# marbl/MHAP

Measured on AMD Instinct MI355X. Metric: overlaps/sec, higher is better.
Workload: dtype int64

## Files before the change

mhap_amd/csrc/kernels.hpp:

```cpp
#pragma once
#include "device_common.hpp"

namespace mhap {

constexpr int HASH_TILE = 1024;
constexpr int WEIGHT_THREADS = 1024;
constexpr int WEIGHT_MAXIT = 24;
constexpr int MH_U = 4;
constexpr int ORD_THREADS = 256;
constexpr int ORD_BINS = 2048;
constexpr int CAND_TQ = 128;
constexpr int CAND_TM = 128;
constexpr int CAND_KS = 32;
constexpr int OVL_THREADS = 128;
#ifndef MH_INV_CT
#define MH_INV_CT 2048
#endif
constexpr int INV_CT = MH_INV_CT;

constexpr int BS_WCLASSES = 6;
constexpr int BS_WMAX = 32;
struct StrandInfo { int32_t valid; int32_t mode; int32_t cnt[BS_WCLASSES + 1]; int32_t pad; };

struct FilterTable {
  const int64_t* keys;
  const double* vals;
  uint32_t mask;
  uint32_t size;
  int32_t enabled;
  int32_t no_tf;
  double range;
  const unsigned long long* bloom; uint64_t bloom_bits; int32_t bloom_k; int32_t bloom_mode;
};

constexpr int META_W = 4;

struct Candidate { int32_t q; int32_t m; };

struct DevRecord { int32_t q, m; double score; int32_t raw, a1, a2, b1, b2, pad; };

struct SearchParams {
  int32_t H, S, k2;
  int32_t num_min_matches, min_store_length;
  int32_t to_self;
  int32_t own_queries;
  double max_shift, threshold;
};

void launch_hash_kmers(hipStream_t st, const ReadDesc* descs, int64_t nstrands, int max_len, const uint8_t* store, int64_t* keys,
                       int32_t* h32, int k, int k2, const uint64_t* luts, int only_mat);
void build_kmer_hash_luts(uint64_t* out);
int weight_grid(int num_cus, int64_t nstrands, int max_len, int k);
bool strand_hashes_from_codes(int length, int k, int k2);
void launch_kmer_weights(hipStream_t st, int num_cus, const ReadDesc* descs, int64_t nstrands, int max_len, const int64_t* keys,
                         uint32_t* wts, uint32_t* perm, uint32_t* slabs, int64_t slab_entries, unsigned long long* counter, int k,
                         const FilterTable& ft, double repeat_weight, StrandInfo* info, bool fused, const uint8_t* store,
                         const uint64_t* luts, const int32_t* order, int32_t* slist);
bool launch_minhash(hipStream_t st, hipStream_t st_weighted, int nblocks, int64_t n_unweighted, int64_t n_weighted, const ReadDesc* descs, int64_t nstrands, const int64_t* keys, const uint32_t* wts,
                    const uint32_t* perm, const StrandInfo* info, const uint8_t* store, const uint64_t* luts, int k, int k2, int H,
                    unsigned long long* counter, int32_t* out_rows, int64_t out_stride, int32_t* out_status, int64_t status_stride,
                    const uint64_t* jump, int jump_na, const int32_t* slist, uint32_t* qbuf, const uint64_t* unjump, const uint64_t* jump_w1, unsigned long long* merge,
                    int max_nk);
size_t minhash_merge_bytes(int nblocks, int H);
void build_xorshift_unjump_tables(int na, int nq, uint64_t* out);
int minhash_wgs_per_cu(int H);
size_t minhash_queue_bytes(int nblocks_total, int H);
int minhash_queue_words(int H);
constexpr int XS_JUMP_LOG2 = 2;
constexpr int XS_JUMP_NQ = BS_WMAX;
#ifndef MH_W1_JUMP_NA
#define MH_W1_JUMP_NA 16
#endif
constexpr int W1_JUMP_NA = MH_W1_JUMP_NA;
inline int w1_jump_tables(int H) { return W1_JUMP_NA + ((H + 1) >> XS_JUMP_LOG2) / W1_JUMP_NA + 1; }
void build_xorshift_jump_tables(int na, int nq, uint64_t* out);
void launch_fix_status(hipStream_t st, int32_t* meta, int64_t nreads);
size_t ordered_lds_bytes(int cap, int code_words, int stage_wide);
void launch_ordered(hipStream_t st, const ReadDesc* descs, int64_t nstrands, int max_len_codes, int max_len, const int32_t* h32,
                    const uint8_t* store, const uint64_t* luts, int k2, int S, int cap, int32_t* out_rows, int64_t out_stride,
                    int32_t* out_meta, int64_t meta_stride, int64_t first = 0, int64_t count = -1);

void launch_candidates(hipStream_t st, const int32_t* minhash, int64_t row_stride, const int32_t* qminhash, int64_t qrow_stride,
                       const int32_t* qlist, int nq, int ne, const int64_t* ids, const int64_t* qids, const int32_t* meta,
                       const int32_t* qmeta, const SearchParams& sp, const long long* rowstart, long long nblocks_tri, Candidate* cand,
                       unsigned long long* cand_count, unsigned long long cand_cap);
constexpr int MHAP_MAX_NUM_HASHES = 8192;
int minhash_waves_per_workgroup(int H);
struct InvIndex {
  uint32_t* ends;
  uint2* items;
  uint32_t nb, shift;
  uint64_t slot_stride;
  uint32_t ne;
  uint32_t grouped;
  uint32_t group_t, class_log;
  uint32_t* lines;
  uint32_t nl_log, line_lb, line_ebits;
  uint32_t tile_entries, tiles;
  uint2* staged;
  uint32_t* tile_counts;
  uint32_t* bin_start;
  uint32_t* bin_long;
};
void launch_query_iota(hipStream_t st, int32_t* qlist, int first, int n);
int index_tile_entries(int ne);
void index_group_params(int64_t entries, InvIndex& ix);
int index_coarse_bins();
bool index_line_params(int64_t entries, uint32_t nb, uint32_t& nl_log, uint32_t& lb, uint32_t& ebits);
size_t index_line_bytes(int H, uint32_t nl_log);
int index_max_buckets_log();
void launch_index_verify(hipStream_t st, const int32_t* minhash, int64_t row_stride, const int32_t* meta, int ne, int H, const InvIndex& ix,
                         unsigned long long* missing);
bool launch_index_build(hipStream_t st, const int32_t* minhash, int64_t row_stride, const int32_t* meta, int ne, int H, const InvIndex& ix);
void launch_index_query(hipStream_t st, const InvIndex& ix, const int32_t* qminhash, int64_t qrow_stride,
                        const int32_t* qlist, int nq, const int64_t* ids, const int64_t* qids, const int32_t* meta, const int32_t* qmeta,
                        const SearchParams& sp, Candidate* cand, unsigned long long* cand_count, unsigned long long cand_cap,
                        unsigned long long* split_count, unsigned long long* elements_total, int32_t* big, unsigned long long* big_count, int tier,
                        unsigned long long* elements_spread);
int index_elements_spread_words();
int index_query_dense_ranges(int64_t entries);
bool index_query_tiers();
bool index_query_tier_ok(int tier, int64_t entries, int num_min_matches);
void oj_stats_dump();
void launch_overlap(hipStream_t st, int nblocks, const Candidate* cand, const unsigned long long* cand_count, unsigned long long cand_cap,
                    const int32_t* ordered, int64_t ord_stride, const int32_t* meta, const int32_t* qordered, int64_t qord_stride,
                    const int32_t* qmeta, const SearchParams& sp, const double* score_table, int32_t* scratch, int64_t scratch_per_lane,
                    DevRecord* recs, unsigned long long* rec_count, unsigned long long rec_cap, unsigned long long* compared, int spread);
constexpr int OJ_MAX_S = 8192;
constexpr int OJ_LEVELS = 3;
constexpr int OJ_GROUP_BAD = 8;
int overlap_join_capacity(int level);
int overlap_join_waves_per_block(int shape);
size_t overlap_join_lds_bytes(int S, int shape, int level);
int overlap_join_blocks_per_cu(int S, int shape, int level);
int overlap_join_table_slots(int S);
void launch_overlap_join(hipStream_t st, int level, int shape, int nblocks, int chunk, const Candidate* cand, const unsigned long long* cand_count,
                         unsigned long long cand_cap, const int32_t* ordered, int64_t ord_stride, const int32_t* meta, const int32_t* qordered,
                         int64_t qord_stride, const int32_t* qmeta, const SearchParams& sp, const double* score_table, DevRecord* recs,
                         unsigned long long* rec_count, unsigned long long rec_cap, unsigned long long* compared, Candidate* slow,
                         unsigned long long* slow_count, unsigned long long* work, const uint16_t* ph = nullptr, const uint16_t* qph = nullptr,
                         const int32_t* pass_min = nullptr);
void launch_poshist(hipStream_t st, const int32_t* ordered, int64_t stride, const int32_t* meta, int64_t n, uint16_t* out);
constexpr int POSHIST_BINS = 64;

}
```

mhap_amd/csrc/mhap_capi.hip:

```cpp
#include <algorithm>
#include <atomic>
#include <cmath>
#include <cstdio>
#include <cstdlib>
#include <chrono>
#include <cstring>
#include <condition_variable>
#include <functional>
#include <mutex>
#include <string>
#include <thread>
#include <vector>

#include "../../include/mhap_hip.h"
static double hp_now() { return std::chrono::duration<double, std::milli>(std::chrono::steady_clock::now().time_since_epoch()).count(); }
#define HPROF(tag) do { if (getenv("MHAP_HOST_PROF")) fprintf(stderr, "[host] %-28s %.3f ms\n", tag, hp_now()); } while (0)
#define DBGSYNC(h, tag) do { if (getenv("MHAP_DEBUG_SYNC")) { fprintf(stderr, "[dbg] %s launched\n", tag); hipError_t _e = hipStreamSynchronize((h)->stream); fprintf(stderr, "[dbg] %s done: %s\n", tag, hipGetErrorString(_e)); } } while (0)
#include "kernels.hpp"
#include "mhap_internal.hpp"
#include "overlap_lane.hpp"

using namespace mhap;

namespace {

struct TimedLaunch { hipEvent_t a, b; int kind; };

inline int64_t align4(int64_t v) { return (v + 3) & ~(int64_t)3; }

void parallel_for(int64_t n, int nthreads, const std::function<void(int64_t, int64_t)>& fn, int64_t grain = 16384) {
  if (n <= 0) return;
  nthreads = (int)std::max<int64_t>(1, std::min<int64_t>(nthreads, n / grain + 1));
  if (nthreads == 1) { fn(0, n); return; }
  std::vector<std::thread> th;
  int64_t chunk = (n + nthreads - 1) / nthreads;
  for (int t = 0; t < nthreads; t++) {
    int64_t lo = t * chunk, hi = std::min(n, lo + chunk);
    if (lo >= hi) break;
    th.emplace_back([=, &fn]() { fn(lo, hi); });
  }
  for (auto& t : th) t.join();
}

void build_bloom(const int64_t* hashes, int64_t n, int64_t size_bloom, std::vector<unsigned long long>& out, uint64_t& bit_size, int& k);

int host_threads() { return usable_host_threads(32); }

}

namespace {
void build_bloom(const int64_t* hashes, int64_t n, int64_t size_bloom, std::vector<unsigned long long>& out, uint64_t& bit_size, int& k) {
  const double nn = (double)(size_bloom <= 0 ? 1 : size_bloom), p = 1.0e-5;
  const int64_t m = (int64_t)(-nn * std::log(p) / (std::log(2.0) * std::log(2.0)));
  k = std::max(1, (int)java_round((double)m / nn * std::log(2.0)));
  const size_t nwords = (size_t)((m + 63) / 64);
  bit_size = (uint64_t)nwords * 64;
  std::vector<std::atomic<unsigned long long>> words(nwords);
  for (auto& w : words) w.store(0ULL, std::memory_order_relaxed);
  const uint64_t bs = bit_size; const int kk = k;
  parallel_for(n, host_threads(), [&](int64_t lo, int64_t hi) {
    for (int64_t i = lo; i < hi; i++) {
      uint64_t h1, h2;
      murmur128_long((uint64_t)hashes[i], h1, h2);
      uint64_t c = h1;
      for (int t = 0; t < kk; t++) {
        const uint64_t bit = (c & 0x7fffffffffffffffULL) % bs;
        words[(size_t)(bit >> 6)].fetch_or(1ULL << (bit & 63), std::memory_order_relaxed);
        c += h2;
      }
    }
  }, 4096);
  out.resize(nwords);
  for (size_t i = 0; i < nwords; i++) out[i] = words[i].load(std::memory_order_relaxed);
}
}

struct mhap_handle {
  mhap_params P;
  int device = 0;
  int num_cus = 256;
  hipStream_t stream = nullptr;
  hipStream_t own_stream = nullptr;
  int oj_per_cu[OJ_LEVELS][3] = {}, oj_per_cu_S = -1;
  int join_mode = 0;
  int join_wide = 2;
  hipStream_t mh_stream = nullptr;
  hipEvent_t ev_mh_fork = nullptr, ev_mh_join = nullptr, ev_ix_fork = nullptr, ev_ix_join = nullptr;
  bool inv_ready = false; int64_t inv_ne = 0;
  uint64_t index_gen = 0;
  bool ph_ready = false; int64_t ph_ne = 0;
  bool iq_start_mid = false;
  int64_t reserve_reads = 0;
  std::string err;
  int Hrow = 1;
  int ord_cap = 0;

  DevBuf f_keys, f_vals, f_bloom;
  FilterTable ft{};
  DevBuf score_tbl, jump_tbl, unjump_tbl, jump_w1_tbl, hash_luts, pass_min_tbl, poshist, q_poshist;

  bool external = false;
  int64_t n_entries = 0;
  DevBuf own_minhash, own_ordered, own_meta;
  int32_t *d_minhash = nullptr, *d_ordered = nullptr, *d_meta = nullptr;
  DevBuf d_ids;
  std::vector<int64_t> ids;
  std::vector<uint8_t> fwd;
  std::vector<int32_t> seqlen;
  std::vector<uint8_t> status;

  DevBuf store, descs, keys, wts, perm, h32, info, slist, slabs, counters, order, mhq, mhmerge;
  int jump_na = 0;
  std::vector<int32_t> h_order;
  uint8_t* pin_store = nullptr;
  size_t pin_cap = 0;
  uint8_t* pin_io = nullptr;
  size_t pin_io_cap = 0;
  ReadDesc* h_descs = nullptr; size_t h_descs_cap = 0;
  struct { int64_t first = 0, n = 0; const int64_t* ids = nullptr; bool done = false; } pend_ids;
  uint64_t mono_gen = ~0ULL; bool mono_val = false, mono_pending = false;
  std::vector<ReadDesc> st_descs;
  std::vector<int64_t> st_ids;
  int64_t st_n = 0, st_bytes = 0;

  DevBuf q_minhash, q_ordered, q_meta, q_ids;

  DevBuf qlist, rowstart, cand, slow_cand, slow_cand2, slow_cand3, recs, recs2, ovl_scratch, inv_ends, inv_items, inv_staged, inv_scratch, inv_big, inv_lines, iq_espread;
  hipStream_t copy_stream = nullptr;
  uint8_t* pin_rec[2] = {nullptr, nullptr};
  size_t pin_rec_cap[2] = {0, 0};
  mhap_record* out_recs2[2] = {nullptr, nullptr};
  size_t out_recs2_cap[2] = {0, 0};
  InvIndex inv{};
  mhap_stage_gate gate = nullptr; void* gate_user = nullptr;
  void* dist = nullptr;
  void* kmer = nullptr;
  std::vector<mhap_record> out_recs;

  std::vector<TimedLaunch> pending;
  std::vector<std::pair<hipEvent_t, hipEvent_t>> free_events;
  mhap_kernel_times ktimes{};
  mhap_stats stats{};
};

namespace {

int fail(mhap_handle* h, int code, const std::string& msg) { h->err = msg; return code; }

#define HIPCHK(h, expr)                                                                              \
  do {                                                                                               \
    hipError_t _e = (expr);                                                                          \
    if (_e != hipSuccess)                                                                            \
      return fail((h), _e == hipErrorOutOfMemory ? MHAP_E_NOMEM : MHAP_E_HIP,                        \
                  std::string(#expr) + ": " + hipGetErrorString(_e));                                \
  } while (0)

size_t time_begin(mhap_handle* h, int kind, hipStream_t st = nullptr) {
  TimedLaunch t; t.kind = kind;
  if (!h->free_events.empty()) { t.a = h->free_events.back().first; t.b = h->free_events.back().second; h->free_events.pop_back(); }
  else { (void)hipEventCreate(&t.a); (void)hipEventCreate(&t.b); }
  (void)hipEventRecord(t.a, st ? st : h->stream);
  h->pending.push_back(t);
  return h->pending.size() - 1;
}
void time_end(mhap_handle* h, hipStream_t st = nullptr) { (void)hipEventRecord(h->pending.back().b, st ? st : h->stream); }
void time_end_at(mhap_handle* h, size_t idx, hipStream_t st = nullptr) { (void)hipEventRecord(h->pending[idx].b, st ? st : h->stream); }

void time_collect(mhap_handle* h) {
  for (auto& t : h->pending) {
    float ms = 0.f;
    if (hipEventElapsedTime(&ms, t.a, t.b) == hipSuccess) { h->ktimes.ms[t.kind] += ms; h->ktimes.launches[t.kind]++; }
    h->free_events.emplace_back(t.a, t.b);
  }
  h->pending.clear();
}

int sync_stream(mhap_handle* h) {
  HIPCHK(h, hipStreamSynchronize(h->stream));
  time_collect(h);
  return MHAP_OK;
}

void build_pass_min(const std::vector<double>& tbl, int S, double threshold, std::vector<int32_t>& pm) {
  pm.assign((size_t)S + 2, INT32_MAX);
  for (int kk = S; kk >= 0; kk--) {
    int32_t best = kk < S ? pm[(size_t)kk + 1] : INT32_MAX;
    for (int it = 0; it <= kk; it++)
      if (tbl[(size_t)score_index(it, kk)] >= threshold) { best = std::min<int32_t>(best, it); break; }
    pm[(size_t)kk] = best;
  }
}
void fill_score_table(int S, int k2, std::vector<double>& tbl) {
  const int64_t n = score_index(S, S) + 1;
  tbl.resize((size_t)n);
  const int64_t half = (S + 2) / 2;
  parallel_for(half, host_threads(), [&](int64_t lo, int64_t hi) {
    auto row = [&](int64_t kk) {
      for (int64_t it = 0; it <= kk; it++) {
        double j = (kk == 0) ? 0.0 : (double)it / (double)kk;
        double d = -1.0 / (double)k2 * std::log(2.0 * j / (1.0 + j));
        tbl[(size_t)score_index((int)it, (int)kk)] = std::exp(-d);
      }
    };
    for (int64_t a = lo; a < hi; a++) { row(a); if (S - a != a && S - a >= half) row(S - a); }
  }, 4);
}

int upload_score_table(mhap_handle* h, const std::vector<double>& tbl, const std::vector<int32_t>& pm) {
  HIPCHK(h, h->score_tbl.ensure(tbl.size() * 8));
  HIPCHK(h, hipMemcpy(h->score_tbl.p, tbl.data(), tbl.size() * 8, hipMemcpyHostToDevice));
  HIPCHK(h, h->pass_min_tbl.ensure(pm.size() * 4));
  HIPCHK(h, hipMemcpy(h->pass_min_tbl.p, pm.data(), pm.size() * 4, hipMemcpyHostToDevice));
  return MHAP_OK;
}

inline int code_of(char c) {
  switch (c) { case 'A': return 0; case 'C': return 1; case 'G': return 2; case 'T': return 3; default: return -1; }
}

static inline uint32_t base_code(uint8_t c) { const uint32_t x = (c >> 1) & 3u; return x ^ (x >> 1); }
static inline bool is_base(uint8_t c) { return ((0x54474341u >> (8 * base_code(c))) & 0xFFu) == c; }

int stage_reads(mhap_handle* h, const char* bases, const int64_t* offsets, const int32_t* lengths, int64_t n, bool fwd_only) {
  HPROF("stage_reads begin");
  const int nthreads = host_threads();
  h->st_descs.resize((size_t)n);
  h->st_n = n;
  std::vector<uint8_t> israw((size_t)n);
  parallel_for(n, nthreads, [&](int64_t lo, int64_t hi) {
    for (int64_t i = lo; i < hi; i++) {
      const uint8_t* s = (const uint8_t*)bases + offsets[i];
      const int L = lengths[i];
      uint32_t bad = 0;
      for (int j = 0; j < L; j++) bad |= is_base(s[j]) ? 0u : 1u;
      israw[(size_t)i] = (uint8_t)bad;
    }
  }, 256);
  int64_t store_bytes = 0;
  for (int64_t i = 0; i < n; i++) {
    ReadDesc& d = h->st_descs[(size_t)i];
    const int L = std::max(0, lengths[i]);
    d.length = L;
    d.flags = 0;
    if (L < h->P.min_olap_length) d.flags |= MHAP_RD_SKIP;
    if (israw[(size_t)i]) d.flags |= MHAP_RD_RAW;
    if (fwd_only) d.flags |= MHAP_RD_FWDONLY;
    d.base_off = store_bytes;
    d.key_off = d.h2_off = 0; d.key_stride = d.h2_stride = 0;
    if (!(d.flags & MHAP_RD_SKIP)) store_bytes += (d.flags & MHAP_RD_RAW) ? align4(L) : align4((L + 3) / 4);
  }
  const size_t need = (size_t)std::max<int64_t>(store_bytes, 4);
  if (h->pin_cap < need) {
    if (h->pin_store) (void)hipHostFree(h->pin_store);
    h->pin_store = nullptr; h->pin_cap = 0;
    HIPCHK(h, hipHostMalloc((void**)&h->pin_store, need + need / 8, hipHostMallocDefault));
    h->pin_cap = need + need / 8;
  }
  uint8_t* hs = h->pin_store;
  parallel_for(n, nthreads, [&](int64_t lo, int64_t hi) {
    for (int64_t i = lo; i < hi; i++) {
      const ReadDesc& d = h->st_descs[(size_t)i];
      if (d.flags & MHAP_RD_SKIP) continue;
      const uint8_t* s = (const uint8_t*)bases + offsets[i];
      uint8_t* dst = hs + d.base_off;
      const int L = d.length;
      if (d.flags & MHAP_RD_RAW) {
        memcpy(dst, s, (size_t)L);
        for (int j = L; j < (int)align4(L); j++) dst[j] = 0;
      } else {
        const int full = L >> 2;
        for (int q = 0; q < full; q++)
          dst[q] = (uint8_t)(base_code(s[4 * q]) | (base_code(s[4 * q + 1]) << 2) | (base_code(s[4 * q + 2]) << 4) | (base_code(s[4 * q + 3]) << 6));
        const int nb = (int)align4((L + 3) / 4);
        for (int q = full; q < nb; q++) {
          uint32_t v = 0;
          for (int j = 4 * q; j < L && j < 4 * q + 4; j++) v |= base_code(s[j]) << (2 * (j & 3));
          dst[q] = (uint8_t)v;
        }
      }
    }
  }, 256);
  HIPCHK(h, h->store.ensure(need));
  HIPCHK(h, hipMemcpyAsync(h->store.p, hs, need, hipMemcpyHostToDevice, h->stream));
  HIPCHK(h, hipStreamSynchronize(h->stream));
  h->st_bytes = (int64_t)need;
  HPROF("stage_reads end (packed + h2d)");
  return MHAP_OK;
}

static int inv_alloc(mhap_handle* h, int64_t ne) {
  const int H = h->P.num_hashes;
  uint32_t lg = 10;
#ifndef MH_INV_BUCKETS_PER_ENTRY
#define MH_INV_BUCKETS_PER_ENTRY 1
#endif
  while (lg < (uint32_t)index_max_buckets_log() && (1ULL << lg) < (uint64_t)MH_INV_BUCKETS_PER_ENTRY * (uint64_t)ne) lg++;
  const int te = index_tile_entries((int)ne);
  const size_t nb = (size_t)1 << lg, stride = (size_t)std::max<int64_t>(ne, 1), tiles = (size_t)((ne + te - 1) / te), cb = (size_t)index_coarse_bins();
  HIPCHK(h, h->inv_ends.ensure((size_t)H * (nb + 1) * 4));
  HIPCHK(h, h->inv_items.ensure((size_t)H * stride * 8));
  HIPCHK(h, h->inv_staged.ensure((size_t)H * stride * 8));
  HIPCHK(h, h->inv_scratch.ensure((size_t)H * (tiles * cb + 2 * cb + 1) * 4));
  h->inv.ends = h->inv_ends.as<uint32_t>(); h->inv.items = h->inv_items.as<uint2>(); h->inv.staged = h->inv_staged.as<uint2>();
  h->inv.tile_counts = h->inv_scratch.as<uint32_t>(); h->inv.bin_start = h->inv.tile_counts + (size_t)H * tiles * cb;
  h->inv.bin_long = h->inv.bin_start + (size_t)H * (cb + 1);
  h->inv.nb = (uint32_t)nb; h->inv.shift = 32 - lg;
  h->inv.slot_stride = (uint64_t)stride;
  h->inv.ne = (uint32_t)std::min<int64_t>(ne, 0xFFFFFFFFLL);
  h->inv.tile_entries = (uint32_t)te; h->inv.tiles = (uint32_t)tiles;
  index_group_params(ne, h->inv);
  h->inv.lines = nullptr; h->inv.nl_log = 0; h->inv.line_lb = 0; h->inv.line_ebits = 0;
  uint32_t nl_log = 0, lb = 0, eb = 0;
  if (index_line_params(ne, (uint32_t)nb, nl_log, lb, eb)) {
    if (h->inv_lines.ensure(index_line_bytes(H, nl_log)) == hipSuccess) {
      h->inv.lines = h->inv_lines.as<uint32_t>(); h->inv.nl_log = nl_log; h->inv.line_lb = lb; h->inv.line_ebits = eb;
    } else (void)hipGetLastError();
  }
  return MHAP_OK;
}

int ensure_inverted_index(mhap_handle* h, hipStream_t st = nullptr, int64_t ne_override = -1);
int fill_ids(mhap_handle* h, int64_t first, const int64_t* ids, int64_t n) {
  h->ids.resize((size_t)(first + 2 * n)); h->fwd.resize((size_t)(first + 2 * n));
  for (int64_t i = 0; i < n; i++) {
    h->ids[(size_t)(first + 2 * i)] = ids[i]; h->ids[(size_t)(first + 2 * i + 1)] = ids[i];
    h->fwd[(size_t)(first + 2 * i)] = 1; h->fwd[(size_t)(first + 2 * i + 1)] = 0;
  }
  HPROF("ids built");
  HIPCHK(h, hipMemcpy(h->d_ids.as<int64_t>() + first, h->ids.data() + first, (size_t)(2 * n) * 8, hipMemcpyHostToDevice));
  HPROF("ids h2d");
  bool mono = true;
  for (int64_t e = 1; e < first + 2 * n && mono; e++) if (h->ids[(size_t)e] < h->ids[(size_t)(e - 1)]) mono = false;
  h->mono_pending = mono;
  return MHAP_OK;
}


int sketch_staged(mhap_handle* h, int32_t* d_minhash, int64_t mh_stride, int32_t* d_ordered, int64_t ord_stride, int32_t* d_meta,
                  int64_t eager_index_entries = 0, bool eager_exchange = false, bool eager_first = false) {
  const int64_t n = h->st_n;
  if (n <= 0) { if (eager_exchange) { const int rx = dist_eager_begin(h, 0, nullptr, false); if (rx < 0) return rx; } return MHAP_OK; }
  HPROF("sketch_staged begin");
  const int k = h->P.kmer_size, k2 = h->P.ordered_kmer_size, H = h->P.num_hashes, S = h->P.ordered_sketch_size;
  int64_t batch_bases = 1LL << 30;
  {
    size_t free_b = 0, total_b = 0;
    if (hipMemGetInfo(&free_b, &total_b) == hipSuccess) {
      const int64_t by_mem = (int64_t)(free_b / 4 / 16);
      batch_bases = std::max<int64_t>(batch_bases, std::min<int64_t>(4LL << 30, by_mem));
    }
  }
  if (const char* e = getenv("MHAP_BATCH_BASES")) { long long v = atoll(e); if (v > 0) batch_bases = v; }
  const char* fenv = getenv("MHAP_FUSED_HASH");
  const bool from_codes_ok = !(fenv && atoi(fenv) == 0);
  auto is_mat = [&](const ReadDesc& d) { return (d.flags & MHAP_RD_RAW) || !from_codes_ok || !strand_hashes_from_codes(d.length, k, k2); };
  struct Batch { int64_t r0, r1; int max_len; };
  std::vector<Batch> plan;
  int64_t max_key = 4, max_h2 = 4, max_w = 4, max_nb = 1;
  int max_len_all = 0;
  for (int64_t r0 = 0; r0 < n;) {
    int64_t r1 = r0, tot = 0;
    while (r1 < n && (r1 == r0 || tot + h->st_descs[(size_t)r1].length <= batch_bases) && (r1 - r0) < (1 << 22)) { tot += h->st_descs[(size_t)r1].length; r1++; }
    Batch b{r0, r1, 0};
    int64_t key_elems = 0, h2_elems = 0, w_elems = 0;
    for (int64_t i = r0; i < r1; i++) {
      const ReadDesc& d = h->st_descs[(size_t)i];
      if (d.flags & MHAP_RD_SKIP) continue;
      w_elems += 2 * align4(std::max(0, d.length - k + 1));
      if (is_mat(d)) { key_elems += 2 * align4(std::max(0, d.length - k + 1)); h2_elems += 2 * align4(std::max(0, d.length - k2 + 1)); }
      b.max_len = std::max(b.max_len, d.length);
    }
    max_key = std::max(max_key, key_elems); max_h2 = std::max(max_h2, h2_elems); max_w = std::max(max_w, w_elems); max_nb = std::max(max_nb, r1 - r0);
    max_len_all = std::max(max_len_all, b.max_len);
    plan.push_back(b);
    r0 = r1;
  }
  bool eager_x = false;
  if (eager_exchange) {
    const int rx = dist_eager_begin(h, n, h->st_ids.data(), plan.size() == 1 && eager_first);
    if (rx < 0) return rx;
    eager_x = rx == 1;
  }
  HIPCHK(h, h->descs.ensure((size_t)max_nb * sizeof(ReadDesc)));
  HIPCHK(h, h->keys.ensure((size_t)max_key * 8));
  HIPCHK(h, h->h32.ensure((size_t)max_h2 * 4));
  HIPCHK(h, h->wts.ensure((size_t)max_w * 4));
  HIPCHK(h, h->perm.ensure((size_t)max_w * 4));
  HIPCHK(h, h->info.ensure((size_t)(2 * max_nb) * sizeof(StrandInfo)));
  HIPCHK(h, h->slist.ensure((size_t)(4 * max_nb) * 4));
  HIPCHK(h, h->counters.ensure(256));
  {
    const int wb = weight_grid(h->num_cus, 2 * max_nb, max_len_all, k);
    int64_t se = 64;
    while (3 * se < 4LL * std::max(1, max_len_all - k + 1)) se <<= 1;
    HIPCHK(h, h->slabs.ensure((size_t)wb * (size_t)se * 4));
  }
  HPROF("sketch: plan + scratch");
  for (const Batch& B : plan) {
    const int64_t nb = B.r1 - B.r0, nstr = 2 * nb;
    if (h->h_descs_cap < (size_t)nb) {
      if (h->h_descs) (void)hipHostFree(h->h_descs);
      h->h_descs = nullptr; h->h_descs_cap = 0;
      const size_t want = (size_t)nb + (size_t)nb / 4 + 64;
      HIPCHK(h, hipHostMalloc((void**)&h->h_descs, want * sizeof(ReadDesc), hipHostMallocDefault));
      h->h_descs_cap = want;
    }
    int64_t key_elems = 0, h2_elems = 0, w_elems = 0;
    bool any_mat = false;
    int min_len_b = INT32_MAX, max_len_codes = 0;
    for (int64_t i = 0; i < nb; i++) {
      ReadDesc d = h->st_descs[(size_t)(B.r0 + i)];
      const bool skip = (d.flags & MHAP_RD_SKIP) != 0;
      if (!skip) min_len_b = std::min(min_len_b, d.length);
      const int64_t nk = align4(std::max(0, d.length - k + 1)), nk2 = align4(std::max(0, d.length - k2 + 1));
      d.key_off = d.h2_off = 0;
      d.w_off = w_elems; d.key_stride = (int32_t)nk; d.h2_stride = (int32_t)nk2;
      if (!skip) {
        w_elems += 2 * nk;
        if (is_mat(d)) {
          d.flags |= MHAP_RD_MAT; any_mat = true;
          d.key_off = key_elems; d.h2_off = h2_elems;
          key_elems += 2 * nk; h2_elems += 2 * nk2;
        } else max_len_codes = std::max(max_len_codes, d.length);
      }
      h->h_descs[(size_t)i] = d;
    }
    const int32_t* d_order = nullptr;
    if (min_len_b * 5 < B.max_len * 4 && nb > 1 && !getenv("MHAP_NO_LENGTH_ORDER")) {
      const int nbk = B.max_len / 128 + 2;
      std::vector<int64_t> start((size_t)nbk + 1, 0);
      for (int64_t i = 0; i < nb; i++) start[(size_t)(nbk - 1 - h->h_descs[(size_t)i].length / 128)]++;
      int64_t acc = 0;
      for (int b = 0; b <= nbk; b++) { const int64_t c = start[(size_t)b]; start[(size_t)b] = acc; acc += c; }
      h->h_order.resize((size_t)nb);
      for (int64_t i = 0; i < nb; i++) h->h_order[(size_t)start[(size_t)(nbk - 1 - h->h_descs[(size_t)i].length / 128)]++] = (int32_t)i;
      HIPCHK(h, h->order.ensure((size_t)nb * 4));
      HIPCHK(h, hipMemcpyAsync(h->order.p, h->h_order.data(), (size_t)nb * 4, hipMemcpyHostToDevice, h->stream));
      d_order = h->order.as<int32_t>();
    }
    int64_t slab_entries = 64;
    while (3 * slab_entries < 4LL * std::max(1, B.max_len - k + 1)) slab_entries <<= 1;
    int32_t* mh_rows = d_minhash + (2 * B.r0) * mh_stride;
    int32_t* ord_rows = d_ordered + (2 * B.r0) * ord_stride;
    int32_t* meta_rows = d_meta + (2 * B.r0) * META_W;
    unsigned long long* ctr = h->counters.as<unsigned long long>();
    const ReadDesc* dd = h->descs.as<ReadDesc>();
    HIPCHK(h, hipMemcpyAsync(h->descs.p, h->h_descs, (size_t)nb * sizeof(ReadDesc), hipMemcpyHostToDevice, h->stream));
    HIPCHK(h, hipMemsetAsync(h->counters.p, 0, 256, h->stream));
    const bool fused = k == 16 && k2 == 12;
    if (any_mat) {
      time_begin(h, MHAP_K_HASH);
      launch_hash_kmers(h->stream, dd, nstr, B.max_len, h->store.as<uint8_t>(), h->keys.as<int64_t>(), h->h32.as<int32_t>(), k, k2,
                        h->hash_luts.as<uint64_t>(), 1);
      time_end(h);
      DBGSYNC(h, "hash_kmers");
    }
    HPROF("sketch: descriptors up");
    time_begin(h, MHAP_K_WEIGHT);
    launch_kmer_weights(h->stream, h->num_cus, dd, nstr, B.max_len, h->keys.as<int64_t>(), h->wts.as<uint32_t>(), h->perm.as<uint32_t>(),
                        h->slabs.as<uint32_t>(), slab_entries, ctr + 0, k, h->ft, h->P.repeat_weight, h->info.as<StrandInfo>(), fused,
                        h->store.as<uint8_t>(), h->hash_luts.as<uint64_t>(), d_order, h->slist.as<int32_t>());
    time_end(h);
    DBGSYNC(h, "kmer_weights");
    int per_cu = minhash_wgs_per_cu(H);
    if (const char* e = getenv("MHAP_MINHASH_WGS_PER_CU")) { int v = atoi(e); if (v >= 1 && v <= 8) per_cu = v; }
    int mblocks = h->num_cus * per_cu;
    if (eager_x) mblocks = std::max(per_cu, mblocks - dist_eager_reserve_wgs(h));
    HIPCHK(h, h->mhq.ensure(minhash_queue_bytes(2 * std::max(mblocks, 1), H) * (size_t)(minhash_waves_per_workgroup(H) < 4 ? 4 : 1)));
    HIPCHK(h, h->mhmerge.ensure(minhash_merge_bytes(std::max(mblocks, 1), H)));
    unsigned long long lens[2] = {0, 0};
    HIPCHK(h, hipMemcpyAsync(lens, ctr + 4, 16, hipMemcpyDeviceToHost, h->stream));
    { const int rs = sync_stream(h); if (rs != MHAP_OK) return rs; }
    HPROF("sketch: list lengths back");
    const hipStream_t ost = h->stream;
    auto do_ordered = [&](int64_t first, int64_t count) -> int {
      time_begin(h, MHAP_K_ORDERED, ost);
      launch_ordered(ost, dd, nstr, max_len_codes, B.max_len, h->h32.as<int32_t>(), h->store.as<uint8_t>(), h->hash_luts.as<uint64_t>(), k2, S, h->ord_cap,
                     ord_rows, ord_stride, meta_rows, META_W, first, count);
      time_end(h, ost);
      return MHAP_OK;
    };
    const int ord_first_env = []() { const char* e = getenv("MHAP_ORDERED_FIRST"); return e ? atoi(e) : 0; }();
    const int ord_split_env = []() { const char* e = getenv("MHAP_ORDERED_SPLIT"); const int v = e ? atoi(e) : -1; return v > 100 ? 100 : v; }();
    int64_t batch_read_bases = 0;
    for (int64_t i = 0; i < nb; i++) batch_read_bases += h->h_descs[(size_t)i].length;
    const bool split_pays = batch_read_bases >= 900000000LL && (int64_t)lens[0] >= 4 * (int64_t)lens[1];
    int64_t ord_pre = ord_first_env ? nstr : (nstr * (int64_t)(ord_split_env >= 0 ? ord_split_env : (split_pays ? 55 : 0))) / 100;
    ord_pre &= ~(int64_t)1;
    bool ordered_done = false;
    if (ord_pre > 0 && !eager_x) {
      (void)do_ordered(0, ord_pre);
      ordered_done = ord_pre >= nstr;
      const int nowait = []() { const char* e = getenv("MHAP_ORDERED_NOWAIT"); return e ? atoi(e) : 1; }();
      if (!nowait) {
        HIPCHK(h, hipEventRecord(h->ev_mh_fork, h->stream));
        HIPCHK(h, hipStreamWaitEvent(h->mh_stream, h->ev_mh_fork, 0));
      }
    } else ord_pre = 0;
    if (eager_x) {
      (void)do_ordered(0, nstr);
      ordered_done = true;
      const int rxo = dist_eager_ordered(h, h->stream, ord_rows);
      if (rxo != MHAP_OK) return rxo;
    }
    {
      const int prefill = []() { const char* e = getenv("MHAP_W1_PREFILL"); return e ? atoi(e) : 0; }();
      if (ord_first_env == 2) (void)hipStreamSynchronize(h->stream);
      for (int i = 0; i < prefill; i++) (void)hipMemsetAsync(h->mhq.p, 0, h->mhq.cap, h->stream);
    }
    const size_t t_mh = time_begin(h, MHAP_K_MINHASH);
    const bool mh_forked = launch_minhash(h->stream, h->mh_stream, mblocks, (int64_t)lens[0], (int64_t)lens[1], dd, nstr, h->keys.as<int64_t>(), h->wts.as<uint32_t>(),
                   h->perm.as<uint32_t>(), h->info.as<StrandInfo>(), h->store.as<uint8_t>(), h->hash_luts.as<uint64_t>(), k, k2, H, ctr, mh_rows, mh_stride,
                   meta_rows + 3, META_W, h->jump_tbl.as<uint64_t>(), h->jump_na, h->slist.as<int32_t>(), h->mhq.as<uint32_t>(), h->unjump_tbl.as<uint64_t>(), h->jump_w1_tbl.as<uint64_t>(),
                   h->mhmerge.as<unsigned long long>(), std::max(0, B.max_len - k + 1));
    if (mh_forked) {
      HIPCHK(h, hipEventRecord(h->ev_mh_join, h->mh_stream));
      HIPCHK(h, hipStreamWaitEvent(h->stream, h->ev_mh_join, 0));
    }
    time_end_at(h, t_mh);
    DBGSYNC(h, "minhash");
    launch_fix_status(h->stream, meta_rows, nb);
    if (eager_x) { const int rxm = dist_eager_minhash(h, h->stream, mh_rows, meta_rows); if (rxm != MHAP_OK) return rxm; }
    bool eager_launched = false;
    if (eager_index_entries > 0 && &B == &plan.back() && !getenv("MHAP_NO_EAGER_INDEX")) {
      HIPCHK(h, hipEventRecord(h->ev_ix_fork, h->stream));
      HIPCHK(h, hipStreamWaitEvent(h->mh_stream, h->ev_ix_fork, 0));
      const int rce = ensure_inverted_index(h, h->mh_stream, eager_index_entries);
      if (rce != MHAP_OK) return rce;
      HIPCHK(h, hipEventRecord(h->ev_ix_join, h->mh_stream));
      eager_launched = true;
    }
    if (!ordered_done) (void)do_ordered(ord_pre, nstr - ord_pre);
    DBGSYNC(h, "ordered");
    HIPCHK(h, hipGetLastError());
    if (eager_launched) HIPCHK(h, hipStreamWaitEvent(h->stream, h->ev_ix_join, 0));
    HPROF("sketch: all launched");
    if (&B == &plan.back() && h->pend_ids.n > 0 && !h->pend_ids.done) {
      const int rf = fill_ids(h, h->pend_ids.first, h->pend_ids.ids, h->pend_ids.n);
      if (rf != MHAP_OK) { (void)sync_stream(h); return rf; }
      h->pend_ids.done = true;
    }
    int rc = sync_stream(h);
    if (rc != MHAP_OK) return rc;
    HPROF("sketch: stream drained");
  }
  return MHAP_OK;
}

int sketch_into(mhap_handle* h, const char* bases, const int64_t* offsets, const int32_t* lengths, int64_t n, bool fwd_only,
                int32_t* d_minhash, int64_t mh_stride, int32_t* d_ordered, int64_t ord_stride, int32_t* d_meta) {
  if (n <= 0) return MHAP_OK;
  int rc = stage_reads(h, bases, offsets, lengths, n, fwd_only);
  if (rc != MHAP_OK) return rc;
  rc = sketch_staged(h, d_minhash, mh_stride, d_ordered, ord_stride, d_meta);
  h->st_n = 0;
  return rc;
}


int ensure_index_capacity(mhap_handle* h, int64_t entries) {
  if (h->external) return fail(h, MHAP_E_STATE, "index tables are externally owned (mhap_index_set_device); clear the index first");
  const int S = h->P.ordered_sketch_size;
  HIPCHK(h, h->own_minhash.ensure((size_t)entries * h->Hrow * 4, true, h->stream));
  HIPCHK(h, h->own_ordered.ensure((size_t)entries * S * 8, true, h->stream));
  HIPCHK(h, h->own_meta.ensure((size_t)entries * META_W * 4, true, h->stream));
  HIPCHK(h, h->d_ids.ensure((size_t)entries * 8, true, h->stream));
  h->d_minhash = h->own_minhash.as<int32_t>();
  h->d_ordered = h->own_ordered.as<int32_t>();
  h->d_meta = h->own_meta.as<int32_t>();
  return MHAP_OK;
}

static void* pinned_io(mhap_handle* h, size_t bytes) {
  if (h->pin_io_cap < bytes) {
    if (h->pin_io) (void)hipHostFree(h->pin_io);
    h->pin_io = nullptr; h->pin_io_cap = 0;
    if (hipHostMalloc((void**)&h->pin_io, bytes + bytes / 4 + 4096, hipHostMallocDefault) != hipSuccess) return nullptr;
    h->pin_io_cap = bytes + bytes / 4 + 4096;
  }
  return h->pin_io;
}

int mirror_meta(mhap_handle* h, const int32_t* d_meta, int64_t first, int64_t count) {
  int32_t* m = (int32_t*)pinned_io(h, (size_t)count * META_W * 4);
  if (!m) return fail(h, MHAP_E_HIP, "cannot allocate pinned host memory");
  HIPCHK(h, hipMemcpy(m, d_meta + first * META_W, (size_t)count * META_W * 4, hipMemcpyDeviceToHost));
  if ((int64_t)h->seqlen.size() < first + count) { h->seqlen.resize((size_t)(first + count)); h->status.resize((size_t)(first + count)); }
  for (int64_t e = 0; e < count; e++) { h->seqlen[(size_t)(first + e)] = m[(size_t)e * META_W + 2]; h->status[(size_t)(first + e)] = (uint8_t)m[(size_t)e * META_W + 3]; }
  return MHAP_OK;
}

struct QuerySide {
  const int32_t* d_minhash; int64_t mh_stride;
  const int32_t* d_ordered; int64_t ord_stride;
  const int32_t* d_meta;
  const int64_t* d_ids;
  const int64_t* h_ids; const int32_t* h_seqlen;
  int64_t n_rows;
  bool identity = false;
  std::function<int(QuerySide&)> prep;
  const uint8_t* h_valid = nullptr;
};

int ensure_inverted_index(mhap_handle* h, hipStream_t st, int64_t ne_override) {
  const int ne = (int)(ne_override >= 0 ? ne_override : h->n_entries), H = h->P.num_hashes;
  if (!st) st = h->stream;
  if (h->inv_ready && h->inv_ne == (int64_t)ne) return MHAP_OK;
  { const int rr = inv_alloc(h, ne); if (rr != MHAP_OK) return rr; }
  HPROF("index build launch");
  time_begin(h, MHAP_K_INDEX_BUILD, st);
  const bool built = launch_index_build(st, h->d_minhash, h->Hrow, h->d_meta, ne, H, h->inv);
  time_end(h, st);
  if (!built) return fail(h, MHAP_E_STATE, "inverted index: its tiles do not cover the entries it was sized for");
  HIPCHK(h, hipGetLastError());
  if (getenv("MHAP_DEBUG_INDEX")) {
    HIPCHK(h, h->counters.ensure(256));
    unsigned long long* ctr = h->counters.as<unsigned long long>();
    unsigned long long missing = 0;
    HIPCHK(h, hipMemsetAsync(ctr + 15, 0, 8, st));
    launch_index_verify(st, h->d_minhash, h->Hrow, h->d_meta, ne, H, h->inv, ctr + 15);
    HIPCHK(h, hipMemcpyAsync(&missing, ctr + 15, 8, hipMemcpyDeviceToHost, st));
    HIPCHK(h, hipStreamSynchronize(st));
    fprintf(stderr, "[index] self-check: %llu of %lld postings missing\n", missing, (long long)ne * H);
    if (missing) return fail(h, MHAP_E_STATE, "inverted index self-check failed");
  }
  h->inv_ready = true; h->inv_ne = ne; h->iq_start_mid = false;
  return MHAP_OK;
}

struct PostStage {
  mhap_handle* h; const QuerySide* qs; mhap_record_sink sink; void* user;
  std::thread th; std::mutex mu; std::condition_variable cv;
  bool started = false, has_job = false, busy = false, stop = false;
  int slot = 0; unsigned long long nrec = 0;
  int rc = MHAP_OK; std::string err; int64_t matches = 0;

  int process(int sl, unsigned long long n) {
    const size_t bytes = (size_t)n * sizeof(DevRecord);
    if (h->pin_rec_cap[sl] < bytes) {
      if (h->pin_rec[sl]) (void)hipHostFree(h->pin_rec[sl]);
      h->pin_rec[sl] = nullptr; h->pin_rec_cap[sl] = 0;
      const size_t want = bytes + bytes / 4 + 4096;
      if (hipHostMalloc((void**)&h->pin_rec[sl], want, hipHostMallocDefault) != hipSuccess) { err = "cannot allocate pinned host memory"; return MHAP_E_HIP; }
      h->pin_rec_cap[sl] = want;
    }
    const DevRecord* hrecs = (const DevRecord*)h->pin_rec[sl];
    const void* src = sl ? h->recs2.p : h->recs.p;
    if (hipMemcpyAsync((void*)hrecs, src, bytes, hipMemcpyDeviceToHost, h->copy_stream) != hipSuccess || hipStreamSynchronize(h->copy_stream) != hipSuccess) {
      err = "record read-back failed"; return MHAP_E_HIP;
    }
    HPROF("tail: records on the host");
    if (h->out_recs2_cap[sl] < (size_t)n) {
      free(h->out_recs2[sl]);
      h->out_recs2_cap[sl] = (size_t)n + (size_t)n / 4 + 1024;
      h->out_recs2[sl] = (mhap_record*)malloc(h->out_recs2_cap[sl] * sizeof(mhap_record));
      if (!h->out_recs2[sl]) { h->out_recs2_cap[sl] = 0; err = "out of host memory (record buffer)"; return MHAP_E_NOMEM; }
    }
    mhap_record* out = h->out_recs2[sl];
    const QuerySide& q = *qs;
    parallel_for((int64_t)n, host_threads(), [&](int64_t lo, int64_t hi) {
      for (int64_t i = lo; i < hi; i++) {
        const DevRecord& d = hrecs[(size_t)i];
        mhap_record& r = out[(size_t)i];
        r.from_id = q.h_ids[d.q]; r.to_id = h->ids[(size_t)d.m];
        r.score = d.score; r.raw = (double)d.raw;
        r.alen = q.h_seqlen[d.q]; r.blen = h->seqlen[(size_t)d.m];
        r.a1 = d.a1; r.a2 = d.a2;
        r.to_rc = h->fwd[(size_t)d.m] ? 0 : 1;
        if (r.to_rc) { r.b1 = r.blen - d.b2 - 1; r.b2 = r.blen - d.b1 - 1; }
        else { r.b1 = d.b1; r.b2 = d.b2; }
        r.pad = 0;
      }
    }, 65536);
    matches += (int64_t)n;
    HPROF("tail: records converted");
    if (sink && sink(out, (int64_t)n, user) != 0) { err = "record sink aborted the search"; return MHAP_E_STATE; }
    HPROF("tail: sink returned");
    return MHAP_OK;
  }
  void loop() {
    (void)hipSetDevice(h->device);
    std::unique_lock<std::mutex> lk(mu);
    for (;;) {
      cv.wait(lk, [&]() { return has_job || stop; });
      if (!has_job) return;
      has_job = false; busy = true;
      const int sl = slot; const unsigned long long n = nrec;
      lk.unlock();
      const int r = rc == MHAP_OK ? process(sl, n) : rc;
      lk.lock();
      if (rc == MHAP_OK) rc = r;
      busy = false;
      cv.notify_all();
    }
  }
  int submit(int sl, unsigned long long n, bool inline_run) {
    if (inline_run && !started) { if (rc == MHAP_OK) rc = process(sl, n); return rc; }
    std::unique_lock<std::mutex> lk(mu);
    if (!started) { started = true; th = std::thread([this]() { loop(); }); }
    cv.wait(lk, [&]() { return !busy && !has_job; });
    if (rc != MHAP_OK) return rc;
    slot = sl; nrec = n; has_job = true;
    cv.notify_all();
    return MHAP_OK;
  }
  int drain() {
    if (started) {
      { std::unique_lock<std::mutex> lk(mu); cv.wait(lk, [&]() { return !busy && !has_job; }); stop = true; cv.notify_all(); }
      th.join(); started = false;
    }
    return rc;
  }
  ~PostStage() { (void)drain(); }
};

int search_core(mhap_handle* h, QuerySide& qs, const std::vector<int32_t>& ql_in, bool to_self, bool triangular_ok,
                mhap_record_sink sink, void* user) {
  const char* cmode = getenv("MHAP_CANDIDATES");
  const bool use_index = !(cmode && strcmp(cmode, "bruteforce") == 0);
  bool prep_done = !qs.prep;
  auto run_prep = [&]() -> int { if (prep_done) return MHAP_OK; prep_done = true; return qs.prep(qs); };
  auto count_valid = [&](int64_t a, int64_t n) { int64_t c = 0; for (int64_t e = a; e < a + n; e++) c += qs.h_valid[(size_t)e] ? 1 : 0; return c; };
  bool ident = qs.identity;
  std::vector<int32_t> ql_made;
  if (ident && (!use_index || h->n_entries == 0 || getenv("MHAP_QUERY_LIST_HOST"))) {
    const int rp = run_prep();
    if (rp != MHAP_OK) return rp;
    ql_made.reserve((size_t)qs.n_rows);
    for (int64_t e = 0; e < qs.n_rows; e++) if (qs.h_valid[(size_t)e]) ql_made.push_back((int32_t)e);
    ident = false;
  }
  const std::vector<int32_t>& ql = qs.identity && !ident ? ql_made : ql_in;
  const int64_t nql = ident ? qs.n_rows : (int64_t)ql.size();
  if (nql == 0 || h->n_entries == 0) { h->stats.queries_searched += nql; return MHAP_OK; }
  const int S = h->P.ordered_sketch_size;
  SearchParams sp;
  sp.H = h->P.num_hashes; sp.S = S; sp.k2 = h->P.ordered_kmer_size;
  sp.num_min_matches = h->P.num_min_matches; sp.min_store_length = h->P.min_store_length; sp.to_self = to_self ? 1 : 0;
  sp.own_queries = (to_self && qs.d_minhash == h->d_minhash && qs.d_meta == h->d_meta && !getenv("MHAP_COUNT_OWN")) ? 1 : 0;
  sp.max_shift = h->P.max_shift; sp.threshold = h->P.threshold;
  const int ne = (int)h->n_entries;
  int64_t qchunk = 262144;
  if (const char* e = getenv("MHAP_QUERY_CHUNK")) { long long v = atoll(e); if (v >= CAND_TQ) qchunk = (v / CAND_TQ) * CAND_TQ; }
  HIPCHK(h, h->qlist.ensure((size_t)nql * 4));
  if (ident) { launch_query_iota(h->stream, h->qlist.as<int32_t>(), 0, (int)nql); HIPCHK(h, hipGetLastError()); }
  else HIPCHK(h, hipMemcpyAsync(h->qlist.p, ql.data(), ql.size() * 4, hipMemcpyHostToDevice, h->stream));
  HIPCHK(h, h->counters.ensure(256));
  unsigned long long* ctr = h->counters.as<unsigned long long>();
  size_t cand_cap = std::max<size_t>(h->cand.cap / sizeof(Candidate), (size_t)4 << 20);
  int64_t ovl_max_blocks = (int64_t)h->num_cus * 16;
  if (const char* e = getenv("MHAP_OVERLAP_BLOCKS")) { long long v = atoll(e); if (v > 0) ovl_max_blocks = v; }
  const int64_t per_lane = 3LL * (2LL * S + 2);
  const char* omode = getenv("MHAP_OVERLAP");
  const bool lane_only = omode && strcmp(omode, "lane") == 0;
  { const char* jw = getenv("MHAP_JOIN_WIDE"); h->join_wide = !jw ? 2 : (jw[0] == '0' ? 0 : (jw[0] == '1' ? 1 : 2)); }
  { const char* jm = getenv("MHAP_JOIN_MODE"); h->join_mode = !jm ? 0 : (strcmp(jm, "alone") == 0 ? 1 : (strcmp(jm, "pair") == 0 ? 2 : (strcmp(jm, "team") == 0 ? 3 : 0))); }
  const int ntu = (ne + CAND_TM - 1) / CAND_TM;
  if (use_index) {
    int rcb = ensure_inverted_index(h);
    if (rcb != MHAP_OK) return rcb;
  }

  h->iq_start_mid = false;
  bool q_ph_done = false;
  PostStage post; post.h = h; post.qs = &qs; post.sink = sink; post.user = user;
#define SCHK(expr) do { const hipError_t _e = (expr); if (_e != hipSuccess) return leave(fail(h, _e == hipErrorOutOfMemory ? MHAP_E_NOMEM : MHAP_E_HIP, std::string(#expr) + ": " + hipGetErrorString(_e))); } while (0)
  auto leave = [&](int code) { const int pr = post.drain(); h->stats.matches_found += post.matches; post.matches = 0;
                               if (code == MHAP_OK && pr != MHAP_OK) return fail(h, pr, post.err); return code; };
  int64_t chunk_no = 0;
  const char* ppe = getenv("MHAP_SEARCH_PIPELINE");
  const bool pipeline = !(ppe && ppe[0] == '0');
  int slot = 0;
  for (int64_t c0 = 0, adv = 0; c0 < nql; c0 += adv, chunk_no++) {
    const int nq = (int)std::min<int64_t>(qchunk, nql - c0);
    adv = nq;
    const int ntq = (nq + CAND_TQ - 1) / CAND_TQ;
    const long long* d_rowstart = nullptr;
    long long nblocks_tri = 0;
    if (triangular_ok && !use_index) {
      std::vector<long long> rs((size_t)ntq + 1);
      long long acc = 0;
      for (int t = 0; t < ntq; t++) {
        rs[(size_t)t] = acc;
        const int32_t maxq = ql[(size_t)(c0 + std::min<int64_t>((int64_t)(t + 1) * CAND_TQ, nq) - 1)];
        acc += std::min<long long>(ntu, ((long long)maxq + CAND_TM - 1) / CAND_TM);
      }
      rs[(size_t)ntq] = acc; nblocks_tri = acc;
      SCHK(h->rowstart.ensure(rs.size() * 8));
      SCHK(hipMemcpyAsync(h->rowstart.p, rs.data(), rs.size() * 8, hipMemcpyHostToDevice, h->stream));
      SCHK(hipStreamSynchronize(h->stream));
      d_rowstart = h->rowstart.as<long long>();
      if (nblocks_tri == 0) { h->stats.queries_searched += nq; continue; }
    }
    unsigned long long ncand = 0;
    for (;;) {
      SCHK(h->cand.ensure(cand_cap * sizeof(Candidate)));
      SCHK(hipMemsetAsync(ctr, 0, 160, h->stream));
      if (use_index) {
        SCHK(h->inv_big.ensure((size_t)nq * 8));
        if (!h->iq_espread.p) { SCHK(h->iq_espread.ensure((size_t)index_elements_spread_words() * 8)); SCHK(hipMemsetAsync(h->iq_espread.p, 0, (size_t)index_elements_spread_words() * 8, h->stream)); }
        unsigned long long* espread = h->iq_espread.as<unsigned long long>();
        const char* tv = getenv("MHAP_INDEX_TIERS");
        const bool tiers = index_query_tiers() && !(tv && tv[0] == '1');
        const char* dv = getenv("MHAP_INDEX_DENSE");
        const bool first_ok = index_query_tier_ok(0, h->n_entries, sp.num_min_matches) && !(dv && dv[0] == '1');
        int32_t* listA = h->inv_big.as<int32_t>();
        int32_t* listB = listA + nq;
        const char* midv = getenv("MHAP_INDEX_MID");
        const bool use_mid = tiers && first_ok && (midv ? midv[0] == '1' : index_query_dense_ranges(h->n_entries) > 4) &&
                             index_query_tier_ok(1, h->n_entries, sp.num_min_matches);
        const int t0 = !first_ok ? 2 : (use_mid && h->iq_start_mid ? 1 : 0);
        time_begin(h, MHAP_K_INDEX_QUERY);
        launch_index_query(h->stream, h->inv, qs.d_minhash, qs.mh_stride, h->qlist.as<int32_t>() + c0, nq,
                           h->d_ids.as<int64_t>(), qs.d_ids, h->d_meta, qs.d_meta, sp, h->cand.as<Candidate>(), ctr + 0,
                           (unsigned long long)cand_cap, ctr + 3, ctr + 4, tiers && t0 < 2 ? listA : nullptr, ctr + 6, t0, espread);
        time_end(h);
        SCHK(hipGetLastError());
        unsigned long long c5[9] = {0, 0, 0, 0, 0, 0, 0, 0, 0};
        SCHK(hipMemcpyAsync(c5, ctr, 72, hipMemcpyDeviceToHost, h->stream));
        if (!prep_done) {
          const int rp = run_prep();
          if (rp != MHAP_OK) { (void)sync_stream(h); return leave(rp); }
          HPROF("query meta on the host");
        }
        int rc = sync_stream(h);
        if (rc != MHAP_OK) return leave(rc);
        HPROF("first query tier done");
        const int32_t* dense_list = listA;
        unsigned long long n_dense = c5[6];
        if (t0 == 0 && use_mid && c5[0] <= cand_cap) {
          if (nq >= 4096 && 2 * c5[6] > (unsigned long long)nq) h->iq_start_mid = true;
          if (c5[6] > 0) {
            time_begin(h, MHAP_K_INDEX_QUERY);
            launch_index_query(h->stream, h->inv, qs.d_minhash, qs.mh_stride, listA, (int)c5[6], h->d_ids.as<int64_t>(), qs.d_ids, h->d_meta, qs.d_meta, sp,
                               h->cand.as<Candidate>(), ctr + 0, (unsigned long long)cand_cap, ctr + 3, ctr + 4, listB, ctr + 8, 1, espread);
            time_end(h);
            SCHK(hipGetLastError());
            SCHK(hipMemcpyAsync(c5, ctr, 72, hipMemcpyDeviceToHost, h->stream));
            rc = sync_stream(h);
            if (rc != MHAP_OK) return leave(rc);
            dense_list = listB; n_dense = c5[8];
          }
        }
        if (n_dense > 0 && c5[0] <= cand_cap) {
          time_begin(h, MHAP_K_INDEX_QUERY);
          launch_index_query(h->stream, h->inv, qs.d_minhash, qs.mh_stride, dense_list, (int)n_dense,
                             h->d_ids.as<int64_t>(), qs.d_ids, h->d_meta, qs.d_meta, sp, h->cand.as<Candidate>(), ctr + 0,
                             (unsigned long long)cand_cap, ctr + 3, ctr + 4, nullptr, nullptr, 2, espread);
          time_end(h);
          SCHK(hipGetLastError());
          SCHK(hipMemcpyAsync(c5, ctr, 72, hipMemcpyDeviceToHost, h->stream));
          rc = sync_stream(h);
          if (rc != MHAP_OK) return leave(rc);
        }
        HPROF("candidates known");
        ncand = c5[0];
        if (ncand <= cand_cap) { h->stats.table_elements += (int64_t)c5[4]; h->stats.index_splits += (int64_t)c5[3]; }
      } else {
        time_begin(h, MHAP_K_CANDIDATE);
        launch_candidates(h->stream, h->d_minhash, h->Hrow, qs.d_minhash, qs.mh_stride, h->qlist.as<int32_t>() + c0, nq, ne,
                          h->d_ids.as<int64_t>(), qs.d_ids, h->d_meta, qs.d_meta, sp, d_rowstart, nblocks_tri, h->cand.as<Candidate>(),
                          ctr + 0, (unsigned long long)cand_cap);
        time_end(h);
        SCHK(hipGetLastError());
        SCHK(hipMemcpyAsync(&ncand, ctr + 0, 8, hipMemcpyDeviceToHost, h->stream));
        int rc = sync_stream(h);
        if (rc != MHAP_OK) return leave(rc);
        if (ncand <= cand_cap) {
          const long long tiles = d_rowstart ? nblocks_tri : (long long)ntq * ntu;
          h->stats.slot_compares += tiles * (long long)CAND_TQ * CAND_TM * sp.H;
        }
      }
      if (ncand <= cand_cap) break;
      cand_cap = (size_t)ncand + (size_t)(ncand / 4) + 1024;
    }
    h->stats.queries_searched += ident ? count_valid(c0, nq) : (int64_t)nq;
    if (ncand == 0) continue;
    if (chunk_no == 0 && (int64_t)ncand >= 64LL * nq && !getenv("MHAP_QUERY_CHUNK")) qchunk = 65536;
    DevBuf& recbuf = slot ? h->recs2 : h->recs;
    SCHK(recbuf.ensure((size_t)ncand * sizeof(DevRecord)));
    if (h->gate && h->gate(h->gate_user) != 0) return leave(fail(h, MHAP_E_STATE, "second-stage gate aborted the search"));
    bool fits[3];
    for (int i = 0; i < 3; i++) fits[i] = overlap_join_lds_bytes(S, i, 0) <= 64 * 1024;
    const bool use_join = !lane_only && S <= OJ_MAX_S && (fits[0] || fits[1] || fits[2]);
    unsigned long long nslow = use_join ? 0 : ncand;
    const Candidate* slow_list = nullptr; unsigned long long* slow_count_ptr = nullptr;
    unsigned long long cj[20] = {0, 0, 0, 0, 0, 0, 0, 0, 0, 0, 0, 0, 0, 0, 0, 0, 0, 0, 0, 0};
    bool have_counts = false;
    if (use_join) {
      SCHK(h->slow_cand.ensure((size_t)ncand * sizeof(Candidate)));
      int shape = (int64_t)ncand >= 4LL * nq ? 2 : ((int64_t)ncand >= 2LL * nq ? 1 : 0);
      if (h->join_mode > 0) shape = h->join_mode - 1;
      while (!fits[shape]) shape = (shape + 1) % 3;
      struct JoinLevel { DevBuf *in, *out; int in_count, out_count, work; };
      const JoinLevel levels[OJ_LEVELS] = {{&h->cand, &h->slow_cand, 0, 5, 7}, {&h->slow_cand, &h->slow_cand2, 5, 10, 9}, {&h->slow_cand2, &h->slow_cand3, 10, 11, 12}};
      struct JoinGrid { int chunk, blocks; };
      auto join_grid = [&](int level, int shp, unsigned long long npairs) {
        if (h->oj_per_cu_S != S) { memset(h->oj_per_cu, 0, sizeof h->oj_per_cu); h->oj_per_cu_S = S; }
        int& per_cu = h->oj_per_cu[level][shp];
        if (per_cu == 0) per_cu = overlap_join_blocks_per_cu(S, shp, level);
        const int wpb = overlap_join_waves_per_block(shp);
        const int64_t resident_waves = (int64_t)h->num_cus * per_cu * wpb;
        JoinGrid g;
        g.chunk = (int)std::max<int64_t>(1, std::min<int64_t>(8, (int64_t)npairs / std::max<int64_t>(resident_waves, 1)));
        const int64_t want = ((int64_t)npairs + (int64_t)wpb * g.chunk - 1) / ((int64_t)wpb * g.chunk);
        g.blocks = (int)std::max<int64_t>(1, std::min<int64_t>((int64_t)h->num_cus * per_cu, want));
        return g;
      };
      const JoinGrid jg = join_grid(0, shape, ncand);
      const char* pe = getenv("MHAP_OVERLAP_PRUNE");
      const bool prune = pe ? pe[0] == '1' : (int64_t)ncand >= 16LL * nq;
      const uint16_t *ph = nullptr, *qph = nullptr;
      if (prune) {
        time_begin(h, MHAP_K_OVERLAP);
        if (!(h->ph_ready && h->ph_ne == h->n_entries)) {
          SCHK(h->poshist.ensure((size_t)h->n_entries * POSHIST_BINS * 2));
          launch_poshist(h->stream, h->d_ordered, 2LL * S, h->d_meta, h->n_entries, h->poshist.as<uint16_t>());
          h->ph_ready = true; h->ph_ne = h->n_entries;
        }
        ph = h->poshist.as<uint16_t>();
        if (qs.d_ordered == h->d_ordered && qs.d_meta == h->d_meta) qph = ph;
        else {
          if (!q_ph_done) {
            SCHK(h->q_poshist.ensure((size_t)qs.n_rows * POSHIST_BINS * 2));
            launch_poshist(h->stream, qs.d_ordered, qs.ord_stride, qs.d_meta, qs.n_rows, h->q_poshist.as<uint16_t>());
            q_ph_done = true;
          }
          qph = h->q_poshist.as<uint16_t>();
        }
        time_end(h);
        SCHK(hipGetLastError());
      }
      time_begin(h, MHAP_K_OVERLAP);
      launch_overlap_join(h->stream, 0, shape, jg.blocks, jg.chunk, h->cand.as<Candidate>(), ctr + levels[0].in_count, (unsigned long long)cand_cap, h->d_ordered, 2LL * S, h->d_meta,
                          qs.d_ordered, qs.ord_stride, qs.d_meta, sp, h->score_tbl.as<double>(), recbuf.as<DevRecord>(), ctr + 1,
                          (unsigned long long)ncand, ctr + 2, h->slow_cand.as<Candidate>(), ctr + levels[0].out_count, ctr + levels[0].work, ph, qph, h->pass_min_tbl.as<int32_t>());
      time_end(h);
      SCHK(hipGetLastError());
      SCHK(hipMemcpyAsync(cj, ctr, 160, hipMemcpyDeviceToHost, h->stream));
      int rcj = sync_stream(h);
      if (rcj != MHAP_OK) return leave(rcj);
      nslow = cj[levels[0].out_count];
      have_counts = nslow == 0;
      unsigned long long group_bad = cj[levels[0].out_count + OJ_GROUP_BAD];
      for (int level = 1; level <= h->join_wide && nslow > 0; level++) {
        if (group_bad * 10 > nslow * 9) break;
        if (overlap_join_lds_bytes(S, 0, level) > 64 * 1024) break;
        const JoinLevel& lv = levels[level];
        SCHK(lv.out->ensure((size_t)nslow * sizeof(Candidate)));
        const JoinGrid wg = join_grid(level, 0, nslow);
        time_begin(h, MHAP_K_OVERLAP);
        launch_overlap_join(h->stream, level, 0, wg.blocks, wg.chunk, lv.in->as<Candidate>(), ctr + lv.in_count, (unsigned long long)ncand, h->d_ordered, 2LL * S, h->d_meta,
                            qs.d_ordered, qs.ord_stride, qs.d_meta, sp, h->score_tbl.as<double>(), recbuf.as<DevRecord>(), ctr + 1, (unsigned long long)ncand, ctr + 2,
                            lv.out->as<Candidate>(), ctr + lv.out_count, ctr + lv.work, nullptr, nullptr, h->pass_min_tbl.as<int32_t>());
        time_end(h);
        SCHK(hipGetLastError());
        unsigned long long cw[20] = {0, 0, 0, 0, 0, 0, 0, 0, 0, 0, 0, 0, 0, 0, 0, 0, 0, 0, 0, 0};
        SCHK(hipMemcpyAsync(cw, ctr, 160, hipMemcpyDeviceToHost, h->stream));
        const int rcw = sync_stream(h);
        if (rcw != MHAP_OK) return leave(rcw);
        for (int i = 0; i < 8; i++) cj[i] = cw[i];
        const unsigned long long before = nslow;
        nslow = cw[lv.out_count];
        group_bad = cw[lv.out_count + OJ_GROUP_BAD];
        slow_list = lv.out->as<Candidate>(); slow_count_ptr = ctr + lv.out_count;
        have_counts = nslow == 0;
        if (nslow * 10 > before * 9) break;
      }
      h->stats.slow_pairs += (int64_t)nslow;
    }
    if (nslow > 0) {
      int spread = 1;
      while (spread < 64 && (int64_t)nslow * spread * 2 <= (int64_t)h->num_cus * 4 * 64) spread *= 2;
      const int oblocks = (int)std::max<int64_t>(1, std::min<int64_t>(ovl_max_blocks, ((int64_t)nslow * spread + OVL_THREADS - 1) / OVL_THREADS));
      SCHK(h->ovl_scratch.ensure((size_t)oblocks * OVL_THREADS / (size_t)spread * (size_t)per_lane * 4));
      time_begin(h, MHAP_K_OVERLAP);
      launch_overlap(h->stream, oblocks, slow_list ? slow_list : (use_join ? h->slow_cand.as<Candidate>() : h->cand.as<Candidate>()), slow_list ? slow_count_ptr : (use_join ? ctr + 5 : ctr + 0),
                     use_join ? (unsigned long long)ncand : (unsigned long long)cand_cap, h->d_ordered, 2LL * S, h->d_meta,
                     qs.d_ordered, qs.ord_stride, qs.d_meta, sp, h->score_tbl.as<double>(), h->ovl_scratch.as<int32_t>(), per_lane,
                     recbuf.as<DevRecord>(), ctr + 1, (unsigned long long)ncand, ctr + 2, spread);
      time_end(h);
      SCHK(hipGetLastError());
    }
    unsigned long long counts[3] = {cj[0], cj[1], cj[2]};
    if (!have_counts) {
      SCHK(hipMemcpyAsync(counts, ctr, 24, hipMemcpyDeviceToHost, h->stream));
      int rc = sync_stream(h);
      if (rc != MHAP_OK) return leave(rc);
    }
    HPROF("overlap done");
    oj_stats_dump();
    const unsigned long long nrec = counts[1];
    h->stats.candidates_compared += (int64_t)counts[2];
    if (nrec == 0) continue;
    const bool last = c0 + nq >= nql;
    const int rp = post.submit(slot, nrec, !pipeline || last);
    if (rp != MHAP_OK) return leave(fail(h, rp, post.err));
    slot ^= 1;
    HPROF("chunk tail handed over");
  }
  return leave(MHAP_OK);
#undef SCHK
}

}

namespace mhap {
HandleView handle_view(mhap_handle* h) {
  HandleView v;
  v.device = h->device; v.stream = h->stream; v.num_cus = h->num_cus; v.Hrow = h->Hrow; v.S = h->P.ordered_sketch_size; v.k = h->P.kmer_size; v.min_olap_length = h->P.min_olap_length;
  v.max_shift = h->P.max_shift;
  v.n_entries = h->n_entries; v.index_gen = h->index_gen;
  v.d_minhash = h->d_minhash; v.d_ordered = h->d_ordered; v.d_meta = h->d_meta;
  v.h_ids = h->ids.data(); v.h_fwd = h->fwd.data(); v.err = &h->err; v.dist = &h->dist; v.kmer = &h->kmer;
  return v;
}
int internal_stage_packed(mhap_handle* h, const ReadDesc* descs, const int64_t* ids, int64_t n, const void* packed, size_t bytes) {
  (void)hipSetDevice(h->device);
  h->st_descs.assign(descs, descs + n);
  h->st_ids.assign(ids, ids + n);
  h->st_n = n;
  const size_t need = std::max<size_t>(bytes, 4);
  HIPCHK(h, h->store.ensure(need));
  if (bytes) HIPCHK(h, hipMemcpyAsync(h->store.p, packed, bytes, hipMemcpyHostToDevice, h->stream));
  HIPCHK(h, hipStreamSynchronize(h->stream));
  h->st_bytes = (int64_t)need;
  return MHAP_OK;
}

int internal_find_matches_device(mhap_handle* h, const void* d_q_minhash, const void* d_q_ordered, const void* d_q_meta, const int64_t* ids,
                                 const int64_t* d_ids_dev, int64_t m, int to_self, mhap_record_sink sink, void* user);

int internal_sketch_queries(mhap_handle* h, const char* bases, const int64_t* offsets, const int32_t* lengths, int64_t n, void* d_mh, void* d_od, void* d_mt) {
  for (int64_t i = 0; i < n; i++) if (lengths[i] < 0) return fail(h, MHAP_E_INVALID, "negative read length");
  return sketch_into(h, bases, offsets, lengths, n, true, (int32_t*)d_mh, h->Hrow, (int32_t*)d_od, 2LL * h->P.ordered_sketch_size, (int32_t*)d_mt);
}
}

extern "C" {

void mhap_default_params(mhap_params* p) {
  p->kmer_size = 16; p->num_hashes = 512; p->ordered_kmer_size = 12; p->ordered_sketch_size = 1536;
  p->num_min_matches = 3; p->min_store_length = 0; p->min_olap_length = 116; p->device = -1;
  p->threshold = 0.78; p->max_shift = 0.2; p->repeat_weight = 0.9;
}

int mhap_create(const mhap_params* params, mhap_handle** out, char* err, size_t errcap) {
  auto seterr = [&](const std::string& m) { if (err && errcap) snprintf(err, errcap, "%s", m.c_str()); };
  if (!params || !out) { seterr("null argument"); return MHAP_E_INVALID; }
  const mhap_params& P = *params;
  if (P.kmer_size < 1 || P.kmer_size > 255) { seterr("k-mer size must be in [1,255]"); return MHAP_E_INVALID; }
  if (P.ordered_kmer_size < 1 || P.ordered_kmer_size > 255) { seterr("ordered k-mer size must be in [1,255]"); return MHAP_E_INVALID; }
  if (P.num_hashes < 1 || P.num_hashes > MHAP_MAX_NUM_HASHES) { seterr("num-hashes must be in [1,8192]"); return MHAP_E_INVALID; }
  if (P.ordered_sketch_size < 1 || P.ordered_sketch_size > 8192) { seterr("ordered-sketch-size must be in [1,8192]"); return MHAP_E_INVALID; }
  if (P.num_min_matches < 1) { seterr("Minimum number of matches must be positive."); return MHAP_E_INVALID; }
  if (P.min_store_length < 0) { seterr("The minimum read length stored must be >=0."); return MHAP_E_INVALID; }
  if (P.max_shift < -1.0) { seterr("The minimum shift must be greater than -1."); return MHAP_E_INVALID; }
  if (P.threshold < 0.0 || P.threshold > 1.0) { seterr("The second stage filter threshold must be 0<=threshold<=1.0."); return MHAP_E_INVALID; }
  HPROF("create begin");
  struct HostTables { std::vector<double> score; std::vector<int32_t> pass_min; std::vector<uint64_t> jump, jump_w1, unjump, luts; int na = 0; } ht;
  std::thread th_score([&]() {
    fill_score_table(P.ordered_sketch_size, P.ordered_kmer_size, ht.score);
    build_pass_min(ht.score, P.ordered_sketch_size, P.threshold, ht.pass_min);
  });
  std::thread th_jump([&]() {
    ht.na = ((P.num_hashes + 1) >> XS_JUMP_LOG2) + 1;
    ht.jump.resize((size_t)(ht.na + XS_JUMP_NQ) * 2048);
    build_xorshift_jump_tables(ht.na, XS_JUMP_NQ, ht.jump.data());
  });
  std::thread th_jump2([&]() {
    const int nt = w1_jump_tables(P.num_hashes);
    ht.jump_w1.resize((size_t)nt * 2048); ht.unjump.resize((size_t)nt * 2048); ht.luts.resize(768);
    build_xorshift_jump_tables(W1_JUMP_NA, nt - W1_JUMP_NA, ht.jump_w1.data());
    build_xorshift_unjump_tables(W1_JUMP_NA, nt - W1_JUMP_NA, ht.unjump.data());
    build_kmer_hash_luts(ht.luts.data());
  });
  struct Join { std::thread& a; std::thread& b; std::thread& c; ~Join() { if (a.joinable()) a.join(); if (b.joinable()) b.join(); if (c.joinable()) c.join(); } } join_tables{th_score, th_jump, th_jump2};
  int ndev = 0;
  hipError_t e = hipGetDeviceCount(&ndev);
  if (e != hipSuccess || ndev <= 0) { seterr(std::string("no HIP device available: ") + hipGetErrorString(e)); return MHAP_E_HIP; }
  mhap_handle* h = new mhap_handle();
  h->P = P;
  int dev = P.device;
  if (dev < 0) { if (hipGetDevice(&dev) != hipSuccess) dev = 0; }
  if (dev >= ndev) { seterr("device ordinal out of range"); delete h; return MHAP_E_INVALID; }
  h->device = dev;
  if ((e = hipSetDevice(dev)) != hipSuccess) { seterr(hipGetErrorString(e)); delete h; return MHAP_E_HIP; }
  hipDeviceProp_t prop;
  h->num_cus = capped_num_cus(hipGetDeviceProperties(&prop, dev) == hipSuccess ? prop.multiProcessorCount : h->num_cus);
  if ((e = hipStreamCreateWithFlags(&h->own_stream, hipStreamNonBlocking)) != hipSuccess) { seterr(hipGetErrorString(e)); delete h; return MHAP_E_HIP; }
  h->stream = h->own_stream;
  if (hipStreamCreateWithFlags(&h->mh_stream, hipStreamNonBlocking) != hipSuccess || hipStreamCreateWithFlags(&h->copy_stream, hipStreamNonBlocking) != hipSuccess ||
      hipEventCreateWithFlags(&h->ev_mh_fork, hipEventDisableTiming) != hipSuccess ||
      hipEventCreateWithFlags(&h->ev_mh_join, hipEventDisableTiming) != hipSuccess || hipEventCreateWithFlags(&h->ev_ix_fork, hipEventDisableTiming) != hipSuccess ||
      hipEventCreateWithFlags(&h->ev_ix_join, hipEventDisableTiming) != hipSuccess) { seterr("cannot create the side streams"); mhap_destroy(h); return MHAP_E_HIP; }
  h->Hrow = std::max(1, P.num_hashes);
  int cap = 1; while (cap < P.ordered_sketch_size) cap <<= 1;
  h->ord_cap = cap;
  h->ft = FilterTable{nullptr, nullptr, 0, 0, 0, 0, 3.0};
  HPROF("create: device + streams");
  th_score.join(); th_jump.join(); th_jump2.join();
  HPROF("create: host tables joined");
  int rc = upload_score_table(h, ht.score, ht.pass_min);
  if (rc != MHAP_OK) { seterr(h->err); mhap_destroy(h); return rc; }
  HPROF("create: score table");
  h->jump_na = ht.na;
  struct Up { DevBuf* b; const std::vector<uint64_t>* v; } ups[] = {{&h->jump_tbl, &ht.jump}, {&h->jump_w1_tbl, &ht.jump_w1}, {&h->unjump_tbl, &ht.unjump}, {&h->hash_luts, &ht.luts}};
  for (const Up& u : ups)
    if (u.b->ensure(u.v->size() * 8) != hipSuccess || hipMemcpy(u.b->p, u.v->data(), u.v->size() * 8, hipMemcpyHostToDevice) != hipSuccess) {
      seterr("cannot allocate the jump / hash tables"); mhap_destroy(h); return MHAP_E_HIP;
    }
  HPROF("create: jump tables");
  *out = h;
  return MHAP_OK;
}

void mhap_destroy(mhap_handle* h) {
  if (!h) return;
  (void)hipSetDevice(h->device);
  if (h->stream) (void)hipStreamSynchronize(h->stream);
  if (h->dist) { mhap_dist_release(h->dist); h->dist = nullptr; }
  if (h->kmer) { kmer_count_release((KmerCountState*)h->kmer); h->kmer = nullptr; }
  for (auto& t : h->pending) { (void)hipEventDestroy(t.a); (void)hipEventDestroy(t.b); }
  for (auto& p : h->free_events) { (void)hipEventDestroy(p.first); (void)hipEventDestroy(p.second); }
  DevBuf* bufs[] = {&h->f_keys, &h->f_vals, &h->f_bloom, &h->score_tbl, &h->jump_tbl, &h->hash_luts, &h->own_minhash, &h->own_ordered, &h->own_meta, &h->d_ids, &h->store, &h->descs,
                    &h->keys, &h->wts, &h->perm, &h->h32, &h->slist, &h->info, &h->slabs, &h->counters, &h->order, &h->mhq, &h->mhmerge, &h->unjump_tbl, &h->jump_w1_tbl, &h->q_minhash, &h->q_ordered, &h->q_meta, &h->q_ids,
                    &h->qlist, &h->rowstart, &h->cand, &h->slow_cand, &h->slow_cand2, &h->slow_cand3, &h->recs, &h->recs2, &h->ovl_scratch, &h->inv_ends, &h->inv_items, &h->inv_staged, &h->inv_scratch, &h->inv_big, &h->inv_lines, &h->iq_espread,
                    &h->pass_min_tbl, &h->poshist, &h->q_poshist};
  for (DevBuf* b : bufs) b->release();
  if (h->pin_store) (void)hipHostFree(h->pin_store);
  if (h->pin_io) (void)hipHostFree(h->pin_io);
  if (h->h_descs) (void)hipHostFree(h->h_descs);
  for (int i = 0; i < 2; i++) { if (h->pin_rec[i]) (void)hipHostFree(h->pin_rec[i]); free(h->out_recs2[i]); }
  if (h->copy_stream) (void)hipStreamDestroy(h->copy_stream);
  if (h->ev_mh_fork) (void)hipEventDestroy(h->ev_mh_fork);
  if (h->ev_mh_join) (void)hipEventDestroy(h->ev_mh_join);
  if (h->ev_ix_fork) (void)hipEventDestroy(h->ev_ix_fork);
  if (h->ev_ix_join) (void)hipEventDestroy(h->ev_ix_join);
  if (h->mh_stream) (void)hipStreamDestroy(h->mh_stream);
  if (h->own_stream) (void)hipStreamDestroy(h->own_stream);
  delete h;
}

const char* mhap_last_error(const mhap_handle* h) { return h ? h->err.c_str() : "null handle"; }

int mhap_set_filter(mhap_handle* h, const int64_t* hashes, const double* fractions, int64_t n, double filter_cutoff, double offset,
                    double range, int no_tf) {
  if (!h) return MHAP_E_INVALID;
  (void)hipSetDevice(h->device);
  if (n <= 0 && !hashes) { h->ft = FilterTable{nullptr, nullptr, 0, 0, 0, 0, range}; return MHAP_OK; }
  if (offset < 0.0 || offset >= 1.0) return fail(h, MHAP_E_INVALID, "Offset can only be between 0 and 1.0.");
  std::vector<int64_t> kk; std::vector<double> ff;
  double maxv = -INFINITY;
  for (int64_t i = 0; i < n; i++) if (fractions[i] >= filter_cutoff) { kk.push_back(hashes[i]); ff.push_back(fractions[i]); maxv = std::max(maxv, fractions[i]); }
  const double minv = filter_cutoff;
  auto idf = [&](double f) { return std::log(maxv / f - offset); };
  const double minIdf = idf(maxv), maxIdf = idf(minv);
  uint32_t ts = 16; while (ts < 2 * kk.size() + 2) ts <<= 1;
  std::vector<int64_t> tk(ts, 0); std::vector<double> tv(ts, 0.0);
  for (size_t i = 0; i < kk.size(); i++) {
    double id = idf(ff[i]);
    double scale = (maxIdf - minIdf) / (double)(range - 1.0);
    double v = 1.0 + (id - minIdf) / scale;
    if (v == 0.0) v = 4.9406564584124654e-324;
    uint32_t slot = (uint32_t)fmix64((uint64_t)kk[i]) & (ts - 1);
    for (;;) {
      if (tv[slot] == 0.0) { tk[slot] = kk[i]; tv[slot] = v; break; }
      if (tk[slot] == kk[i]) { tv[slot] = v; break; }
      slot = (slot + 1) & (ts - 1);
    }
  }
  HIPCHK(h, h->f_keys.ensure((size_t)ts * 8));
  HIPCHK(h, h->f_vals.ensure((size_t)ts * 8));
  HIPCHK(h, hipMemcpy(h->f_keys.p, tk.data(), (size_t)ts * 8, hipMemcpyHostToDevice));
  HIPCHK(h, hipMemcpy(h->f_vals.p, tv.data(), (size_t)ts * 8, hipMemcpyHostToDevice));
  h->ft.keys = h->f_keys.as<int64_t>(); h->ft.vals = h->f_vals.as<double>();
  h->ft.mask = ts - 1; h->ft.size = (uint32_t)kk.size(); h->ft.enabled = 1; h->ft.no_tf = no_tf ? 1 : 0; h->ft.range = range;
  h->ft.bloom = nullptr; h->ft.bloom_bits = 0; h->ft.bloom_k = 0; h->ft.bloom_mode = 0;
  return MHAP_OK;
}

int mhap_set_filter_whitelist(mhap_handle* h, const int64_t* hashes, int64_t n, int64_t size_bloom, int32_t mode) {
  if (!h) return MHAP_E_INVALID;
  if (mode < 0 || mode > 2) return fail(h, MHAP_E_INVALID, "Unknown removeUnique option.");
  if (mode == 0) { h->ft.bloom = nullptr; h->ft.bloom_bits = 0; h->ft.bloom_k = 0; h->ft.bloom_mode = 0; return MHAP_OK; }
  if (!h->ft.enabled) return fail(h, MHAP_E_STATE, "set the k-mer filter (mhap_set_filter) before its whitelist");
  if (n < 0 || (n > 0 && !hashes) || size_bloom < 0) return fail(h, MHAP_E_INVALID, "bad whitelist arguments");
  (void)hipSetDevice(h->device);
  std::vector<unsigned long long> words;
  uint64_t bit_size = 0; int k = 0;
  build_bloom(hashes, n, size_bloom, words, bit_size, k);
  const size_t nwords = words.size();
  HIPCHK(h, h->f_bloom.ensure(nwords * 8));
  HIPCHK(h, hipMemcpy(h->f_bloom.p, words.data(), nwords * 8, hipMemcpyHostToDevice));
  h->ft.bloom = h->f_bloom.as<unsigned long long>(); h->ft.bloom_bits = bit_size; h->ft.bloom_k = k; h->ft.bloom_mode = mode;
  return MHAP_OK;
}

static int finish_add(mhap_handle* h, int64_t first, const int64_t* ids, int64_t n);

static int leave_collective_add(mhap_handle* h, int code) {
  if (h->dist != nullptr && dist_eager_wanted(h)) {
    const std::string keep = h->err;
    const int rx = dist_eager_begin(h, 0, nullptr, false);
    if (code != MHAP_OK) h->err = keep;
    else if (rx < 0) return rx;
  }
  return code;
}

int mhap_index_add_reads(mhap_handle* h, const char* bases, const int64_t* offsets, const int32_t* lengths, const int64_t* ids, int64_t n) {
  if (!h) return MHAP_E_INVALID;
  (void)hipSetDevice(h->device);
  if (n > 0 && (!bases || !offsets || !lengths || !ids)) return leave_collective_add(h, fail(h, MHAP_E_INVALID, "null argument"));
  if (n <= 0) return leave_collective_add(h, MHAP_OK);
  if (h->n_entries + 2 * n > (int64_t)INT32_MAX / 2) return leave_collective_add(h, fail(h, MHAP_E_INVALID, "index too large for 32-bit entry indices"));
  for (int64_t i = 0; i < n; i++) if (lengths[i] < 0) return leave_collective_add(h, fail(h, MHAP_E_INVALID, "negative read length"));
  int rc = mhap_stage_reads(h, bases, offsets, lengths, ids, n);
  if (rc != MHAP_OK) return leave_collective_add(h, rc);
  rc = mhap_index_add_staged(h);
  h->st_n = 0;
  return rc;
}

static int finish_add(mhap_handle* h, int64_t first, const int64_t* ids, int64_t n) {
  HPROF("finish_add begin");
  const bool early = h->pend_ids.done && h->pend_ids.first == first && h->pend_ids.n == n && h->pend_ids.ids == ids;
  h->pend_ids.done = false; h->pend_ids.n = 0;
  auto undo = [&](int code) { h->ids.resize((size_t)first); h->fwd.resize((size_t)first); return code; };
  if (!early) { const int rf = fill_ids(h, first, ids, n); if (rf != MHAP_OK) return undo(rf); }
  h->inv_ready = false; h->ph_ready = false;
  int rc = mirror_meta(h, h->d_meta, first, 2 * n);
  HPROF("meta mirrored");
  if (rc != MHAP_OK) return undo(rc);
  h->index_gen++;
  h->mono_val = h->mono_pending; h->mono_gen = h->index_gen;
  h->n_entries = first + 2 * n;
  h->stats.strands_indexed = 0;
  for (int64_t e = 0; e < h->n_entries; e++) if (h->status[(size_t)e] == 0) h->stats.strands_indexed++;
  return MHAP_OK;
}

int mhap_stage_reads(mhap_handle* h, const char* bases, const int64_t* offsets, const int32_t* lengths, const int64_t* ids, int64_t n) {
  if (!h || n < 0 || (n > 0 && (!bases || !offsets || !lengths || !ids))) return h ? fail(h, MHAP_E_INVALID, "null argument") : MHAP_E_INVALID;
  (void)hipSetDevice(h->device);
  for (int64_t i = 0; i < n; i++) if (lengths[i] < 0) return fail(h, MHAP_E_INVALID, "negative read length");
  h->st_ids.assign(ids, ids + n);
  if (n == 0) { h->st_n = 0; return MHAP_OK; }
  return stage_reads(h, bases, offsets, lengths, n, false);
}

int mhap_index_reserve(mhap_handle* h, int64_t total_reads) {
  if (!h || total_reads < 0) return h ? fail(h, MHAP_E_INVALID, "negative read count") : MHAP_E_INVALID;
  if (h->n_entries != 0) return fail(h, MHAP_E_STATE, "mhap_index_reserve applies to an empty index");
  if (2 * total_reads > (int64_t)INT32_MAX / 2) return fail(h, MHAP_E_INVALID, "index too large for 32-bit entry indices");
  h->reserve_reads = total_reads;
  return MHAP_OK;
}

int mhap_index_add_staged(mhap_handle* h) {
  if (!h) return MHAP_E_INVALID;
  (void)hipSetDevice(h->device);
  const int64_t n = h->st_n;
  if (n <= 0 || (int64_t)h->st_ids.size() != n) return leave_collective_add(h, fail(h, MHAP_E_STATE, "no staged reads (call mhap_stage_reads first)"));
  if (h->n_entries + 2 * n > (int64_t)INT32_MAX / 2) return leave_collective_add(h, fail(h, MHAP_E_INVALID, "index too large for 32-bit entry indices"));
  const int64_t first = h->n_entries;
  const int64_t want_entries = std::max<int64_t>(first + 2 * n, first == 0 ? 2 * h->reserve_reads : 0);
  int rc = ensure_index_capacity(h, want_entries);
  if (rc != MHAP_OK) return leave_collective_add(h, rc);
  const int S = h->P.ordered_sketch_size;
  h->ph_ready = false; h->inv_ready = false;
  const int64_t after = first + 2 * n;
  const bool likely_last = (first == 0 && 2 * h->reserve_reads <= after) || (h->reserve_reads > 0 && after == 2 * h->reserve_reads);
  const bool eager_exchange = h->dist != nullptr && dist_eager_wanted(h);
  h->pend_ids.first = first; h->pend_ids.n = n; h->pend_ids.ids = h->st_ids.data(); h->pend_ids.done = false;
  rc = sketch_staged(h, h->d_minhash + first * h->Hrow, h->Hrow, h->d_ordered + first * 2LL * S, 2LL * S, h->d_meta + first * META_W,
                     likely_last ? after : 0, eager_exchange, first == 0);
  if (rc != MHAP_OK) {
    h->pend_ids.n = 0; h->pend_ids.done = false;
    h->ids.resize((size_t)first); h->fwd.resize((size_t)first);
    return rc;
  }
  const bool built = h->inv_ready && h->inv_ne == after;
  rc = finish_add(h, first, h->st_ids.data(), n);
  if (rc == MHAP_OK && built) h->inv_ready = true;
  if (rc == MHAP_OK && eager_exchange) dist_eager_commit(h);
  return rc;
}

int mhap_sketch_staged_device(mhap_handle* h, void* d_minhash, void* d_ordered, void* d_meta) {
  if (!h || !d_minhash || !d_ordered || !d_meta) return h ? fail(h, MHAP_E_INVALID, "null argument") : MHAP_E_INVALID;
  (void)hipSetDevice(h->device);
  if (h->st_n <= 0) return fail(h, MHAP_E_STATE, "no staged reads (call mhap_stage_reads first)");
  return sketch_staged(h, (int32_t*)d_minhash, h->Hrow, (int32_t*)d_ordered, 2LL * h->P.ordered_sketch_size, (int32_t*)d_meta);
}

int mhap_sketch_batch(mhap_handle* h, const char* bases, const int64_t* offsets, const int32_t* lengths, int64_t n, int32_t* minhash,
                      int32_t* ordered, int32_t* ordered_size, uint8_t* status) {
  if (!h) return MHAP_E_INVALID;
  if (n <= 0) return MHAP_OK;
  if (!bases || !offsets || !lengths) return fail(h, MHAP_E_INVALID, "null argument");
  (void)hipSetDevice(h->device);
  const int S = h->P.ordered_sketch_size;
  HIPCHK(h, h->q_minhash.ensure((size_t)(2 * n) * h->Hrow * 4));
  HIPCHK(h, h->q_ordered.ensure((size_t)(2 * n) * S * 8));
  HIPCHK(h, h->q_meta.ensure((size_t)(2 * n) * META_W * 4));
  int rc = sketch_into(h, bases, offsets, lengths, n, false, h->q_minhash.as<int32_t>(), h->Hrow, h->q_ordered.as<int32_t>(), 2LL * S,
                       h->q_meta.as<int32_t>());
  if (rc != MHAP_OK) return rc;
  std::vector<int32_t> meta((size_t)(2 * n) * META_W);
  HIPCHK(h, hipMemcpy(meta.data(), h->q_meta.p, meta.size() * 4, hipMemcpyDeviceToHost));
  if (minhash) HIPCHK(h, hipMemcpy(minhash, h->q_minhash.p, (size_t)(2 * n) * h->Hrow * 4, hipMemcpyDeviceToHost));
  if (ordered) HIPCHK(h, hipMemcpy(ordered, h->q_ordered.p, (size_t)(2 * n) * S * 8, hipMemcpyDeviceToHost));
  for (int64_t e = 0; e < 2 * n; e++) {
    if (ordered_size) ordered_size[e] = meta[(size_t)e * META_W + 3] == 0 ? meta[(size_t)e * META_W + 0] : 0;
    if (status) status[e] = (uint8_t)meta[(size_t)e * META_W + 3];
  }
  return MHAP_OK;
}

static bool ordered_positions_ok(const int32_t* ordered, const int32_t* ordered_size, const int32_t* ordered_seqlen, int64_t m, int S, int64_t* bad_entry) {
  std::atomic<int64_t> bad{-1};
  parallel_for(m, host_threads(), [&](int64_t lo, int64_t hi) {
    for (int64_t e = lo; e < hi && bad.load(std::memory_order_relaxed) < 0; e++) {
      const int32_t n = ordered_size[e], len = ordered_seqlen[e];
      if (n < 0 || n > S) continue;
      const int32_t* row = ordered + (size_t)e * (size_t)S * 2;
      uint32_t out = 0;
      for (int32_t i = 0; i < n; i++) out |= (uint32_t)((uint32_t)row[2 * i + 1] >= (uint32_t)len);
      if (out) { int64_t want = -1; bad.compare_exchange_strong(want, e); }
    }
  }, 256);
  *bad_entry = bad.load();
  return *bad_entry < 0;
}

int mhap_index_add_sketches(mhap_handle* h, const int64_t* ids, const uint8_t* is_fwd, const int32_t* seq_length, const int32_t* minhash,
                            const int32_t* ordered, const int32_t* ordered_size, const int32_t* ordered_seqlen, int64_t m) {
  if (!h) return MHAP_E_INVALID;
  if (m <= 0) return MHAP_OK;
  if (!ids || !is_fwd || !seq_length || !minhash || !ordered || !ordered_size || !ordered_seqlen) return fail(h, MHAP_E_INVALID, "null argument");
  (void)hipSetDevice(h->device);
  if (h->n_entries + m > (int64_t)INT32_MAX / 2) return fail(h, MHAP_E_INVALID, "index too large for 32-bit entry indices");
  for (int64_t e = 0; e < m; e++)
    if (seq_length[e] < 0 || ordered_seqlen[e] < 0) return fail(h, MHAP_E_INVALID, "negative sequence length in a precomputed sketch");
  {
    int64_t bad = -1;
    if (!ordered_positions_ok(ordered, ordered_size, ordered_seqlen, m, h->P.ordered_sketch_size, &bad))
      return fail(h, MHAP_E_INVALID, "precomputed sketch " + std::to_string(bad) + ": an ordered-sketch position outside [0, its sequence's k-mer count)");
  }
  int rc = ensure_index_capacity(h, h->n_entries + m);
  if (rc != MHAP_OK) return rc;
  const int64_t first = h->n_entries;
  const int S = h->P.ordered_sketch_size;
  std::vector<int32_t> meta((size_t)m * META_W);
  for (int64_t e = 0; e < m; e++) {
    if (ordered_size[e] < 0 || ordered_size[e] > S) return fail(h, MHAP_E_INVALID, "ordered sketch larger than --ordered-sketch-size");
    meta[(size_t)e * META_W + 0] = ordered_size[e]; meta[(size_t)e * META_W + 1] = ordered_seqlen[e];
    meta[(size_t)e * META_W + 2] = seq_length[e]; meta[(size_t)e * META_W + 3] = 0;
  }
  HIPCHK(h, hipMemcpy(h->d_minhash + first * h->Hrow, minhash, (size_t)m * h->Hrow * 4, hipMemcpyHostToDevice));
  HIPCHK(h, hipMemcpy(h->d_ordered + first * 2LL * S, ordered, (size_t)m * S * 8, hipMemcpyHostToDevice));
  HIPCHK(h, hipMemcpy(h->d_meta + first * META_W, meta.data(), meta.size() * 4, hipMemcpyHostToDevice));
  h->ids.resize((size_t)(first + m)); h->fwd.resize((size_t)(first + m));
  for (int64_t e = 0; e < m; e++) { h->ids[(size_t)(first + e)] = ids[e]; h->fwd[(size_t)(first + e)] = is_fwd[e] ? 1 : 0; }
  HIPCHK(h, hipMemcpy(h->d_ids.as<int64_t>() + first, h->ids.data() + first, (size_t)m * 8, hipMemcpyHostToDevice));
  rc = mirror_meta(h, h->d_meta, first, m);
  if (rc != MHAP_OK) return rc;
  h->n_entries = first + m; h->inv_ready = false; h->ph_ready = false; h->index_gen++;
  h->stats.strands_indexed += m;
  return MHAP_OK;
}

int mhap_index_size(mhap_handle* h, int64_t* entries) {
  if (!h || !entries) return MHAP_E_INVALID;
  *entries = h->n_entries;
  return MHAP_OK;
}

int mhap_index_export(mhap_handle* h, int64_t first, int64_t count, int64_t* ids, uint8_t* is_fwd, int32_t* seq_length, int32_t* minhash,
                      int32_t* ordered, int32_t* ordered_size, int32_t* ordered_seqlen, uint8_t* status) {
  if (!h) return MHAP_E_INVALID;
  if (first < 0 || count < 0 || first + count > h->n_entries) return fail(h, MHAP_E_INVALID, "export range outside the index");
  if (count == 0) return MHAP_OK;
  (void)hipSetDevice(h->device);
  const int S = h->P.ordered_sketch_size;
  std::vector<int32_t> meta((size_t)count * META_W);
  HIPCHK(h, hipMemcpy(meta.data(), h->d_meta + first * META_W, meta.size() * 4, hipMemcpyDeviceToHost));
  if (minhash) HIPCHK(h, hipMemcpy(minhash, h->d_minhash + first * h->Hrow, (size_t)count * h->Hrow * 4, hipMemcpyDeviceToHost));
  if (ordered) HIPCHK(h, hipMemcpy(ordered, h->d_ordered + first * 2LL * S, (size_t)count * S * 8, hipMemcpyDeviceToHost));
  for (int64_t e = 0; e < count; e++) {
    if (ids) ids[e] = h->ids[(size_t)(first + e)];
    if (is_fwd) is_fwd[e] = h->fwd[(size_t)(first + e)];
    if (seq_length) seq_length[e] = meta[(size_t)e * META_W + 2];
    if (ordered_size) ordered_size[e] = meta[(size_t)e * META_W + 0];
    if (ordered_seqlen) ordered_seqlen[e] = meta[(size_t)e * META_W + 1];
    if (status) status[e] = (uint8_t)meta[(size_t)e * META_W + 3];
  }
  return MHAP_OK;
}

int mhap_index_clear(mhap_handle* h) {
  if (!h) return MHAP_E_INVALID;
  h->n_entries = 0; h->external = false; h->inv_ready = false; h->ph_ready = false; h->reserve_reads = 0; h->index_gen++;
  h->ids.clear(); h->fwd.clear(); h->seqlen.clear(); h->status.clear();
  h->d_minhash = h->own_minhash.as<int32_t>(); h->d_ordered = h->own_ordered.as<int32_t>(); h->d_meta = h->own_meta.as<int32_t>();
  h->stats = mhap_stats{};
  return MHAP_OK;
}

int mhap_index_prepare(mhap_handle* h) {
  if (!h) return MHAP_E_INVALID;
  (void)hipSetDevice(h->device);
  if (h->n_entries == 0) return MHAP_OK;
  const int rc = ensure_inverted_index(h);
  if (rc != MHAP_OK) return rc;
  return sync_stream(h);
}

int mhap_sketch_reads_device(mhap_handle* h, const char* bases, const int64_t* offsets, const int32_t* lengths, int64_t n, void* d_minhash,
                             void* d_ordered, void* d_meta) {
  if (!h) return MHAP_E_INVALID;
  if (n <= 0) return MHAP_OK;
  if (!bases || !offsets || !lengths || !d_minhash || !d_ordered || !d_meta) return fail(h, MHAP_E_INVALID, "null argument");
  (void)hipSetDevice(h->device);
  return sketch_into(h, bases, offsets, lengths, n, false, (int32_t*)d_minhash, h->Hrow, (int32_t*)d_ordered, 2LL * h->P.ordered_sketch_size,
                     (int32_t*)d_meta);
}

int mhap_index_set_device(mhap_handle* h, const int64_t* ids, const uint8_t* is_fwd, void* d_minhash, void* d_ordered, void* d_meta, int64_t m) {
  if (!h) return MHAP_E_INVALID;
  if (m < 0 || (m > 0 && (!ids || !is_fwd || !d_minhash || !d_ordered || !d_meta))) return fail(h, MHAP_E_INVALID, "null argument");
  if (m > (int64_t)INT32_MAX / 2) return fail(h, MHAP_E_INVALID, "index too large for 32-bit entry indices");
  (void)hipSetDevice(h->device);
  mhap_index_clear(h);
  h->external = true;
  h->d_minhash = (int32_t*)d_minhash; h->d_ordered = (int32_t*)d_ordered; h->d_meta = (int32_t*)d_meta;
  h->ids.assign(ids, ids + m); h->fwd.assign(is_fwd, is_fwd + m);
  HIPCHK(h, h->d_ids.ensure((size_t)std::max<int64_t>(m, 1) * 8));
  if (m > 0) HIPCHK(h, hipMemcpy(h->d_ids.p, ids, (size_t)m * 8, hipMemcpyHostToDevice));
  if (m > 0) { int rc = mirror_meta(h, h->d_meta, 0, m); if (rc != MHAP_OK) return rc; }
  h->n_entries = m; h->inv_ready = false; h->ph_ready = false; h->index_gen++;
  for (int64_t e = 0; e < m; e++) if (h->status[(size_t)e] == 0) h->stats.strands_indexed++;
  return MHAP_OK;
}

static int self_search(mhap_handle* h, int64_t q_first, int64_t q_count, int64_t shard, int64_t nshards, mhap_record_sink sink, void* user) {
  HPROF("self_search begin");
  (void)hipSetDevice(h->device);
  if (q_first < 0 || q_first > h->n_entries) return fail(h, MHAP_E_INVALID, "query range outside the index");
  if (nshards < 1 || shard < 0 || shard >= nshards) return fail(h, MHAP_E_INVALID, "bad shard");
  int64_t q_end = (q_count < 0) ? h->n_entries : std::min(h->n_entries, q_first + q_count);
  std::vector<int32_t> ql;
  int64_t ordinal = 0;
  for (int64_t e = 0; e < q_end; e++) {
    if (!h->fwd[(size_t)e]) continue;
    const int64_t o = ordinal++;
    if (e < q_first || (o % nshards) != shard) continue;
    if (h->status[(size_t)e] == 0) ql.push_back((int32_t)e);
  }
  bool mono = true;
  if (h->mono_gen == h->index_gen) mono = h->mono_val;
  else for (int64_t e = 1; e < h->n_entries && mono; e++) if (h->ids[(size_t)e] < h->ids[(size_t)(e - 1)]) mono = false;
  const bool tri = mono && h->P.min_store_length == 0 && !getenv("MHAP_NO_TRIANGULAR");
  QuerySide qs{h->d_minhash, h->Hrow, h->d_ordered, 2LL * h->P.ordered_sketch_size, h->d_meta, h->d_ids.as<int64_t>(), h->ids.data(), h->seqlen.data(), h->n_entries};
  HPROF("search_core begin");
  const int rcs = search_core(h, qs, ql, true, tri, sink, user);
  HPROF("search_core end");
  return rcs;
}

int mhap_find_matches_self(mhap_handle* h, int64_t q_first, int64_t q_count, mhap_record_sink sink, void* user) {
  if (!h) return MHAP_E_INVALID;
  return self_search(h, q_first, q_count, 0, 1, sink, user);
}

int mhap_find_matches_self_shard(mhap_handle* h, int64_t shard, int64_t nshards, mhap_record_sink sink, void* user) {
  if (!h) return MHAP_E_INVALID;
  return self_search(h, 0, -1, shard, nshards, sink, user);
}

int mhap_find_matches_reads(mhap_handle* h, const char* bases, const int64_t* offsets, const int32_t* lengths, const int64_t* ids, int64_t n,
                            mhap_record_sink sink, void* user) {
  if (!h) return MHAP_E_INVALID;
  if (n <= 0) return MHAP_OK;
  if (!bases || !offsets || !lengths || !ids) return fail(h, MHAP_E_INVALID, "null argument");
  (void)hipSetDevice(h->device);
  const int S = h->P.ordered_sketch_size;
  HIPCHK(h, h->q_minhash.ensure((size_t)(2 * n) * h->Hrow * 4));
  HIPCHK(h, h->q_ordered.ensure((size_t)(2 * n) * S * 8));
  HIPCHK(h, h->q_meta.ensure((size_t)(2 * n) * META_W * 4));
  HIPCHK(h, h->q_ids.ensure((size_t)(2 * n) * 8));
  int rc = sketch_into(h, bases, offsets, lengths, n, true, h->q_minhash.as<int32_t>(), h->Hrow, h->q_ordered.as<int32_t>(), 2LL * S,
                       h->q_meta.as<int32_t>());
  if (rc != MHAP_OK) return rc;
  std::vector<int32_t> meta((size_t)(2 * n) * META_W);
  HIPCHK(h, hipMemcpy(meta.data(), h->q_meta.p, meta.size() * 4, hipMemcpyDeviceToHost));
  std::vector<int64_t> qids((size_t)(2 * n));
  std::vector<int32_t> qlen((size_t)(2 * n));
  std::vector<int32_t> ql;
  for (int64_t i = 0; i < n; i++) {
    qids[(size_t)(2 * i)] = qids[(size_t)(2 * i + 1)] = ids[i];
    qlen[(size_t)(2 * i)] = qlen[(size_t)(2 * i + 1)] = lengths[i];
    if (meta[(size_t)(2 * i) * META_W + 3] == 0) ql.push_back((int32_t)(2 * i));
  }
  HIPCHK(h, hipMemcpy(h->q_ids.p, qids.data(), qids.size() * 8, hipMemcpyHostToDevice));
  QuerySide qs{h->q_minhash.as<int32_t>(), h->Hrow, h->q_ordered.as<int32_t>(), 2LL * S, h->q_meta.as<int32_t>(), h->q_ids.as<int64_t>(),
               qids.data(), qlen.data(), 2 * n};
  return search_core(h, qs, ql, false, false, sink, user);
}

int mhap_find_matches_sketches(mhap_handle* h, const int64_t* ids, const int32_t* seq_length, const int32_t* minhash, const int32_t* ordered,
                               const int32_t* ordered_size, const int32_t* ordered_seqlen, int64_t m, mhap_record_sink sink, void* user) {
  if (!h) return MHAP_E_INVALID;
  if (m <= 0) return MHAP_OK;
  if (!ids || !seq_length || !minhash || !ordered || !ordered_size || !ordered_seqlen) return fail(h, MHAP_E_INVALID, "null argument");
  (void)hipSetDevice(h->device);
  const int S = h->P.ordered_sketch_size;
  for (int64_t e = 0; e < m; e++)
    if (seq_length[e] < 0 || ordered_seqlen[e] < 0) return fail(h, MHAP_E_INVALID, "negative sequence length in a precomputed sketch");
  {
    int64_t bad = -1;
    if (!ordered_positions_ok(ordered, ordered_size, ordered_seqlen, m, S, &bad))
      return fail(h, MHAP_E_INVALID, "query sketch " + std::to_string(bad) + ": an ordered-sketch position outside [0, its sequence's k-mer count)");
  }
  std::vector<int32_t> meta((size_t)m * META_W);
  std::vector<int32_t> ql((size_t)m);
  for (int64_t e = 0; e < m; e++) {
    if (ordered_size[e] < 0 || ordered_size[e] > S) return fail(h, MHAP_E_INVALID, "ordered sketch larger than --ordered-sketch-size");
    meta[(size_t)e * META_W + 0] = ordered_size[e]; meta[(size_t)e * META_W + 1] = ordered_seqlen[e];
    meta[(size_t)e * META_W + 2] = seq_length[e]; meta[(size_t)e * META_W + 3] = 0;
    ql[(size_t)e] = (int32_t)e;
  }
  HIPCHK(h, h->q_minhash.ensure((size_t)m * h->Hrow * 4));
  HIPCHK(h, h->q_ordered.ensure((size_t)m * S * 8));
  HIPCHK(h, h->q_meta.ensure((size_t)m * META_W * 4));
  HIPCHK(h, h->q_ids.ensure((size_t)m * 8));
  HIPCHK(h, hipMemcpy(h->q_minhash.p, minhash, (size_t)m * h->Hrow * 4, hipMemcpyHostToDevice));
  HIPCHK(h, hipMemcpy(h->q_ordered.p, ordered, (size_t)m * S * 8, hipMemcpyHostToDevice));
  HIPCHK(h, hipMemcpy(h->q_meta.p, meta.data(), meta.size() * 4, hipMemcpyHostToDevice));
  HIPCHK(h, hipMemcpy(h->q_ids.p, ids, (size_t)m * 8, hipMemcpyHostToDevice));
  QuerySide qs{h->q_minhash.as<int32_t>(), h->Hrow, h->q_ordered.as<int32_t>(), 2LL * S, h->q_meta.as<int32_t>(), h->q_ids.as<int64_t>(), ids,
               seq_length, m};
  return search_core(h, qs, ql, false, false, sink, user);
}

static int find_matches_device_impl(mhap_handle* h, const void* d_q_minhash, const void* d_q_ordered, const void* d_q_meta, const int64_t* ids,
                                    const int64_t* d_ids_dev, int64_t m, int to_self, mhap_record_sink sink, void* user) {
  if (!h) return MHAP_E_INVALID;
  if (m <= 0) return MHAP_OK;
  if (!d_q_minhash || !d_q_ordered || !d_q_meta || !ids) return fail(h, MHAP_E_INVALID, "null argument");
  if (m > (int64_t)INT32_MAX / 2) return fail(h, MHAP_E_INVALID, "too many query rows");
  (void)hipSetDevice(h->device);
  const int S = h->P.ordered_sketch_size;
  const size_t mbytes = (size_t)m * META_W * 4, idbytes = d_ids_dev ? 0 : (size_t)m * 8;
  char* pin = (char*)pinned_io(h, mbytes + idbytes);
  if (!pin) return fail(h, MHAP_E_HIP, "cannot allocate pinned host memory");
  const int32_t* meta = (const int32_t*)pin;
  if (!d_ids_dev) {
    HIPCHK(h, h->q_ids.ensure((size_t)m * 8));
    memcpy(pin + mbytes, ids, idbytes);
    HIPCHK(h, hipMemcpyAsync(h->q_ids.p, pin + mbytes, idbytes, hipMemcpyHostToDevice, h->stream));
  }
  HIPCHK(h, hipMemcpyAsync((void*)meta, d_q_meta, mbytes, hipMemcpyDeviceToHost, h->copy_stream));
  std::vector<int32_t> qlen((size_t)m), ql;
  std::vector<uint8_t> valid((size_t)m);
  QuerySide qs{(const int32_t*)d_q_minhash, h->Hrow, (const int32_t*)d_q_ordered, 2LL * S, (const int32_t*)d_q_meta,
               d_ids_dev ? d_ids_dev : h->q_ids.as<int64_t>(), ids, qlen.data(), m};
  qs.identity = true;
  qs.prep = [&](QuerySide& q) -> int {
    const hipError_t e = hipStreamSynchronize(h->copy_stream);
    if (e != hipSuccess) return fail(h, MHAP_E_HIP, std::string("read-back of the query rows' meta words: ") + hipGetErrorString(e));
    for (int64_t i = 0; i < m; i++) { qlen[(size_t)i] = meta[(size_t)i * META_W + 2]; valid[(size_t)i] = meta[(size_t)i * META_W + 3] == 0 ? 1 : 0; }
    q.h_valid = valid.data();
    return MHAP_OK;
  };
  const int rcs = search_core(h, qs, ql, to_self != 0, false, sink, user);
  if (qs.prep) (void)hipStreamSynchronize(h->copy_stream);
  return rcs;
}

int mhap_find_matches_device(mhap_handle* h, const void* d_q_minhash, const void* d_q_ordered, const void* d_q_meta, const int64_t* ids,
                             int64_t m, int to_self, mhap_record_sink sink, void* user) {
  return find_matches_device_impl(h, d_q_minhash, d_q_ordered, d_q_meta, ids, nullptr, m, to_self, sink, user);
}

int mhap_set_second_stage_gate(mhap_handle* h, mhap_stage_gate gate, void* user) {
  if (!h) return MHAP_E_INVALID;
  h->gate = gate; h->gate_user = user;
  return MHAP_OK;
}

int mhap_get_stats(mhap_handle* h, mhap_stats* out) { if (!h || !out) return MHAP_E_INVALID; *out = h->stats; return MHAP_OK; }
int mhap_get_kernel_times(mhap_handle* h, mhap_kernel_times* out) { if (!h || !out) return MHAP_E_INVALID; *out = h->ktimes; return MHAP_OK; }
int mhap_reset_kernel_times(mhap_handle* h) { if (!h) return MHAP_E_INVALID; h->ktimes = mhap_kernel_times{}; return MHAP_OK; }
int mhap_set_stream(mhap_handle* h, void* hip_stream) {
  if (!h) return MHAP_E_INVALID;
  (void)hipSetDevice(h->device);
  (void)hipStreamSynchronize(h->stream);
  h->stream = hip_stream ? (hipStream_t)hip_stream : h->own_stream;
  return MHAP_OK;
}
int mhap_synchronize(mhap_handle* h) { if (!h) return MHAP_E_INVALID; (void)hipSetDevice(h->device); return sync_stream(h); }

}

extern "C" {

int mhap_hash_kmer(const char* kmer, int32_t len, int32_t do_rc, int64_t* out) {
  if (!kmer || !out || len < 1 || len > 4096) return MHAP_E_INVALID;
  std::string s(kmer, (size_t)len);
  if (do_rc) {
    std::string r((size_t)len, 'N');
    for (int i = 0; i < len; i++) r[(size_t)i] = (char)rc_char((uint32_t)(uint8_t)s[(size_t)(len - 1 - i)]);
    if (r.compare(s) < 0) s = r;
  }
  std::vector<uint32_t> W((size_t)len / 4 + 3, 0u);
  memcpy(W.data(), s.data(), (size_t)len);
  *out = (int64_t)murmur128_h1_chars<0>(W.data(), 0, len);
  return MHAP_OK;
}

int mhap_selftest_hash_windows(const char* seq, int32_t len, int32_t k, int32_t k2, int64_t* out64, int32_t* out32) {
  if (!seq || len < 0 || k < 1 || k2 < 1) return MHAP_E_INVALID;
  std::vector<uint32_t> W((size_t)len / 4 + 3, 0u);
  memcpy(W.data(), seq, (size_t)len);
  if (out64) for (int p = 0; p + k <= len; p++) out64[p] = (k == 16) ? (int64_t)murmur128_h1_chars<16>(W.data(), p, k) : (int64_t)murmur128_h1_chars<0>(W.data(), p, k);
  if (out32) for (int p = 0; p + k2 <= len; p++) out32[p] = (k2 == 12) ? (int32_t)murmur32_chars<12>(W.data(), p, k2) : (int32_t)murmur32_chars<0>(W.data(), p, k2);
  return MHAP_OK;
}

int mhap_selftest_xorshift_jump(uint64_t key, int32_t nsteps, uint64_t* out) {
  if (!out || nsteps < 0 || nsteps > (1 << 16)) return MHAP_E_INVALID;
  const int a = nsteps >> XS_JUMP_LOG2, r = nsteps & ((1 << XS_JUMP_LOG2) - 1);
  uint64_t x = key;
  if (a > 0) {
    const int na = a < 24 ? a : 24;
    int qa = 0, af = a;
    if (af > na) { qa = (af - 1) / na; af -= qa * na; }
    std::vector<uint64_t> jt((size_t)(na + qa + 1) * 2048);
    build_xorshift_jump_tables(na, qa + 1, jt.data());
    if (qa > 0) {
      const uint64_t* T = jt.data() + (size_t)(na + qa - 1) * 2048;
      uint64_t y = 0;
      for (int i = 0; i < 8; i++) y ^= T[i * 256 + (int)((x >> (8 * i)) & 255u)];
      x = y;
    }
    const uint64_t* T = jt.data() + (size_t)(af - 1) * 2048;
    uint64_t y = 0;
    for (int i = 0; i < 8; i++) y ^= T[i * 256 + (int)((x >> (8 * i)) & 255u)];
    x = y;
  }
  for (int t = 0; t < r; t++) x = xorshift_step(x);
  *out = x;
  return MHAP_OK;
}

int mhap_selftest_xorshift_unjump(uint64_t x, int32_t nsteps, uint64_t* out) {
  if (!out || nsteps < 1 || nsteps > (1 << 15)) return MHAP_E_INVALID;
  int a = (nsteps + (1 << XS_JUMP_LOG2) - 1) >> XS_JUMP_LOG2;
  const int r = (a << XS_JUMP_LOG2) - nsteps;
  const int qa = a > W1_JUMP_NA ? (a - 1) / W1_JUMP_NA : 0;
  a -= qa * W1_JUMP_NA;
  std::vector<uint64_t> ut((size_t)(W1_JUMP_NA + qa) * 2048);
  build_xorshift_unjump_tables(W1_JUMP_NA, qa, ut.data());
  uint64_t y = x;
  if (qa > 0) {
    const uint64_t* T = ut.data() + (size_t)(W1_JUMP_NA + qa - 1) * 2048;
    uint64_t z = 0;
    for (int i = 0; i < 8; i++) z ^= T[i * 256 + (int)((y >> (8 * i)) & 255u)];
    y = z;
  }
  {
    const uint64_t* T = ut.data() + (size_t)(a - 1) * 2048;
    uint64_t z = 0;
    for (int i = 0; i < 8; i++) z ^= T[i * 256 + (int)((y >> (8 * i)) & 255u)];
    y = z;
  }
  for (int t = 0; t < r; t++) y = xorshift_step(y);
  *out = y;
  return MHAP_OK;
}

int mhap_selftest_bloom(const int64_t* hashes, int64_t n, int64_t size_bloom, const int64_t* probes, int64_t np, uint8_t* out_flags, int64_t* out2) {
  if ((n > 0 && !hashes) || (np > 0 && (!probes || !out_flags)) || !out2) return MHAP_E_INVALID;
  std::vector<unsigned long long> words; uint64_t bit_size = 0; int k = 0;
  build_bloom(hashes, n, size_bloom, words, bit_size, k);
  for (int64_t i = 0; i < np; i++) out_flags[i] = bloom_might_contain(words.data(), bit_size, k, (uint64_t)probes[i]) ? 1 : 0;
  out2[0] = (int64_t)bit_size; out2[1] = k;
  return MHAP_OK;
}

int mhap_selftest_pass_min(int32_t S, int32_t k2, double threshold, double* scores, int32_t* pass_min) {
  if (S < 1 || S > 8192 || k2 < 1 || !pass_min) return MHAP_E_INVALID;
  std::vector<double> tbl; std::vector<int32_t> pm;
  fill_score_table(S, k2, tbl);
  build_pass_min(tbl, S, threshold, pm);
  if (scores) memcpy(scores, tbl.data(), tbl.size() * 8);
  memcpy(pass_min, pm.data(), pm.size() * 4);
  return MHAP_OK;
}

int mhap_selftest_transpose32(uint32_t* a32) {
  if (!a32) return MHAP_E_INVALID;
  uint32_t a[32];
  memcpy(a, a32, sizeof a);
  transpose32(a);
  memcpy(a32, a, sizeof a);
  return MHAP_OK;
}

int mhap_selftest_overlap_lane(const int32_t* A, int32_t nA, int32_t lenA, const int32_t* B, int32_t nB, int32_t lenB, double max_shift,
                               int32_t stride, int32_t* out8) {
  if (!A || !B || !out8 || stride < 1) return MHAP_E_INVALID;
  const int maxrec = 2 * std::max(nA, nB) + 2;
  std::vector<int32_t> scratch((size_t)3 * (size_t)maxrec * (size_t)stride, 0);
  LaneScratch sc; sc.base = scratch.data(); sc.stride = stride; sc.maxrec = maxrec;
  PlainView va{A, nA}, vb{B, nB};
  const LaneOverlap r = lane_overlap(va, lenA, vb, lenB, max_shift, sc);
  out8[0] = r.empty; out8[1] = r.valid; out8[2] = r.a1; out8[3] = r.a2; out8[4] = r.b1; out8[5] = r.b2; out8[6] = r.inter; out8[7] = r.kk;
  return MHAP_OK;
}

}

namespace mhap {
int internal_find_matches_device(mhap_handle* h, const void* d_q_minhash, const void* d_q_ordered, const void* d_q_meta, const int64_t* ids,
                                 const int64_t* d_ids_dev, int64_t m, int to_self, mhap_record_sink sink, void* user) {
  return find_matches_device_impl(h, d_q_minhash, d_q_ordered, d_q_meta, ids, d_ids_dev, m, to_self, sink, user);
}
}
```

mhap_amd/csrc/sketch_kernels.hip:

```cpp
#include <cstdlib>
#include <cstring>

#include "kernels.hpp"
#include <algorithm>
#ifdef MH_ORD_PATHS
#include <cstdio>
#include <string>
#include <vector>
#endif

namespace mhap {

constexpr int HASH_SEG = 4096;
constexpr int HASH_LUT_WORDS = 3 * 256;

void build_kmer_hash_luts(uint64_t* out) {
  const uint64_t c1 = 0x87c37b91114253d5ULL, c2 = 0x4cf5ad432745937fULL;
  const uint32_t d1 = 0xcc9e2d51U, d2 = 0x1b873593U;
  const char* acgt = "ACGT";
  for (int idx = 0; idx < 256; idx++) {
    uint64_t block = 0;
    for (int c = 0; c < 4; c++) block |= (uint64_t)(uint8_t)acgt[(idx >> (2 * c)) & 3] << (16 * c);
    uint64_t k1 = block * c1; k1 = rotl64(k1, 31); k1 *= c2;
    uint64_t k2 = block * c2; k2 = rotl64(k2, 33); k2 *= c1;
// ... 1907 lines not shown
#pragma unroll
    for (int q = 0; q < 3; q++) {
      const uint64_t kk = lut[(cw >> (8 * q)) & 255u];
      h ^= (uint32_t)kk;         h = rotl32(h, 13); h = mm3_mul5c(h);
      h ^= (uint32_t)(kk >> 32); h = rotl32(h, 13); h = mm3_mul5c(h);
    }
    h ^= 24u;
    return (int32_t)fmix32(h);
  };
  const int K = S < n ? S : n;
  if (threadIdx.x == 0) { meta[0] = K; meta[1] = n; meta[2] = rd.length; }
  if (K <= 0) return;
  ORD_PATH_VARS;

  const double ksig = sqrt((double)K), csig = sqrt((double)cap);
  const double target = fmin((double)K + 7.0 * ksig, (double)cap - 5.0 * csig);
  if (n > cap && target >= (double)K + 3.0 * ksig) {
    const double quant = target / (double)n;
    const uint32_t cut_u = quant >= 1.0 ? 0xFFFFFFFFu : (uint32_t)(quant * 4294967296.0);
    const uint32_t cutbin = cut_u >> 21;
    for (uint32_t j = threadIdx.x; j < ORD_BINS; j += ORD_THREADS) hist[j] = 0;
    if (threadIdx.x == 0) { s_fill = 0; s_cnt = 0; }
    __syncthreads();
    const int lane = threadIdx.x & 63;
    for (int ib = 0; ib < n; ib += 8 * ORD_THREADS) {
      const int p0 = ib + 32 * (int)(threadIdx.x >> 2) + (int)(threadIdx.x & 3);
      int32_t hv[8];
      if (mat) {
#pragma unroll
        for (int u = 0; u < 8; u++) { const int i = p0 + 4 * u; hv[u] = i < n ? hp[i] : 0; }
      } else if (p0 < n) {
        const int d = p0 >> 4;
        const uint32_t sh = (uint32_t)(2 * (p0 & 15));
        const uint32_t w0 = codes[d], w1 = codes[d + 1], w2 = codes[d + 2], w3 = codes[d + 3];
        const uint32_t a[3] = {__builtin_amdgcn_alignbit(w1, w0, sh), __builtin_amdgcn_alignbit(w2, w1, sh), __builtin_amdgcn_alignbit(w3, w2, sh)};
        uint64_t g[10];
#pragma unroll
        for (int j = 0; j < 10; j++) g[j] = lut[(a[j >> 2] >> (8 * (j & 3))) & 255u];
#pragma unroll
        for (int u = 0; u < 8; u++) {
          uint32_t h = 0;
#pragma unroll
          for (int q = 0; q < 3; q++) {
            const uint64_t kk = g[u + q];
            h ^= (uint32_t)kk;         h = rotl32(h, 13); h = mm3_mul5c(h);
            h ^= (uint32_t)(kk >> 32); h = rotl32(h, 13); h = mm3_mul5c(h);
          }
          h ^= 24u;
          hv[u] = (int32_t)fmix32(h);
        }
      } else {
#pragma unroll
        for (int u = 0; u < 8; u++) hv[u] = 0;
      }
      unsigned long long bal[8];
      uint32_t total = 0;
#pragma unroll
      for (int u = 0; u < 8; u++) {
        bal[u] = __ballot(p0 + 4 * u < n && ((uint32_t)hv[u] ^ 0x80000000u) < cut_u);
        total += (uint32_t)__popcll(bal[u]);
      }
      if (total) {
        uint32_t base = 0;
        if (lane == 0) base = atomicAdd(&s_fill, total);
        base = (uint32_t)__builtin_amdgcn_readfirstlane((int)base);
#pragma unroll
        for (int u = 0; u < 8; u++) {
          if ((bal[u] >> lane) & 1ULL) {
            const uint32_t idx = base + __builtin_amdgcn_mbcnt_hi((uint32_t)(bal[u] >> 32), __builtin_amdgcn_mbcnt_lo((uint32_t)bal[u], 0u));
            if (idx < (uint32_t)cap) { if (stage_wide) stage[idx] = (uint32_t)(p0 + 4 * u); else stage16[idx] = (uint16_t)(p0 + 4 * u); }
            atomicAdd(&hist[((uint32_t)hv[u] ^ 0x80000000u) >> 21], 1u);
          }
          base += (uint32_t)__popcll(bal[u]);
        }
      }
    }
    __syncthreads();
    ORD_TICK(1);
    const uint32_t m = s_fill;
    bool ok = m >= (uint32_t)K && m <= (uint32_t)cap;
    ORD_PATH_ATT(m < (uint32_t)K ? 2 : m > (uint32_t)cap ? 3 : 1);
    if (ok) {
      const int per = ORD_BINS / ORD_THREADS;
      uint32_t loc = 0, mx = 0;
      for (int j = 0; j < per; j++) { const uint32_t c = hist[threadIdx.x * per + j]; loc += c; mx = c > mx ? c : mx; }
      uint32_t incl = loc;
#pragma unroll
      for (int off = 1; off < 64; off <<= 1) { const uint32_t v = __shfl_up(incl, off); if (lane >= off) incl += v; }
      if (lane == 63) part[threadIdx.x >> 6] = incl;
      if (mx > ORD_BUCKET_MAX) atomicMax(&s_cnt, mx);
      __syncthreads();
      for (unsigned w = 0; w < (threadIdx.x >> 6); w++) incl += part[w];
      uint32_t run = incl - loc;
      for (int j = 0; j < per; j++) { const uint32_t b = threadIdx.x * per + j; bstart[b] = (uint16_t)run; run += hist[b]; }
      ok = s_cnt == 0;
      __syncthreads();
      if (!ok) ORD_PATH_ATT(4);
    }
    ORD_TICK(2);
    if (ok) {
      for (uint32_t b = threadIdx.x; b <= cutbin; b += ORD_THREADS) hist[b] = 0;
      __syncthreads();
      for (uint32_t t0 = threadIdx.x; t0 < m; t0 += 4 * ORD_THREADS) {
        int ii[4]; uint64_t key[4]; uint32_t slot[4];
#pragma unroll
        for (int u = 0; u < 4; u++) { const uint32_t t = t0 + (uint32_t)u * ORD_THREADS; ii[u] = t < m ? (stage_wide ? (int)stage[t] : (int)stage16[t]) : 0; }
#pragma unroll
        for (int u = 0; u < 4; u++) key[u] = okey(hget(ii[u]), ii[u]);
#pragma unroll
        for (int u = 0; u < 4; u++) { const uint32_t b = (uint32_t)(key[u] >> 53); slot[u] = t0 + (uint32_t)u * ORD_THREADS < m ? (uint32_t)bstart[b] + atomicAdd(&hist[b], 1u) : 0xFFFFFFFFu; }
#pragma unroll
        for (int u = 0; u < 4; u++) if (slot[u] != 0xFFFFFFFFu) buf[slot[u]] = key[u];
      }
      __syncthreads();
      ORD_TICK(3);
      int32_t* orow = out_rows + strand * out_stride;
      for (uint32_t t0 = threadIdx.x; t0 < m; t0 += 2 * ORD_THREADS) {
        uint64_t key[2]; uint32_t s0[2], c[2], rank[2] = {0u, 0u};
#pragma unroll
        for (int u = 0; u < 2; u++) {
          const uint32_t t = t0 + (uint32_t)u * ORD_THREADS;
          key[u] = buf[t < m ? t : t0];
          const uint32_t b = (uint32_t)(key[u] >> 53);
          s0[u] = bstart[b]; c[u] = t < m ? hist[b] : 0u;
        }
        const uint32_t cmax = c[0] > c[1] ? c[0] : c[1];
        for (uint32_t q = 0; q < cmax; q += 4) {
          uint64_t o[2][4];
#pragma unroll
          for (int u = 0; u < 2; u++)
#pragma unroll
            for (int x = 0; x < 4; x++) o[u][x] = buf[s0[u] + q + (uint32_t)x < (uint32_t)cap ? s0[u] + q + (uint32_t)x : s0[u]];
#pragma unroll
          for (int u = 0; u < 2; u++)
#pragma unroll
            for (int x = 0; x < 4; x++) rank[u] += (q + (uint32_t)x < c[u] && o[u][x] < key[u]) ? 1u : 0u;
        }
#pragma unroll
        for (int u = 0; u < 2; u++) {
          const uint32_t j = s0[u] + rank[u];
          if (t0 + (uint32_t)u * ORD_THREADS < m && j < (uint32_t)K) { orow[2 * j] = (int32_t)((uint32_t)(key[u] >> 32) ^ 0x80000000u); orow[2 * j + 1] = (int32_t)(uint32_t)key[u]; }
        }
      }
      ORD_TICK(5);
#ifdef MH_ORD_PROF
      if (threadIdx.x == 0) atomicAdd(&g_ord_prof[7], 1ULL);
#endif
      ORD_PATH_HOW(2);
      return;
    }
    __syncthreads();
  }

  uint64_t bound = ~0ULL;
  bool buckets = false;
  uint32_t bk_bin = 0, bk_total = 0;
  if (threadIdx.x == 0) s_fill = 0;
  if (n > cap) {
    const int shifts[6] = {53, 42, 32, 21, 10, 0};
    const int widths[6] = {11, 11, 10, 11, 11, 10};
    uint64_t prefix = 0;
    uint64_t prefmask = 0;
    uint32_t below = 0;
    for (int lv = 0; lv < 6; lv++) {
      const int sh = shifts[lv];
      const uint32_t nb = 1u << widths[lv];
      for (uint32_t j = threadIdx.x; j < ORD_BINS; j += ORD_THREADS) hist[j] = 0;
      __syncthreads();
      for (int i0 = threadIdx.x; i0 < n; i0 += 8 * ORD_THREADS) {
        int32_t hv[8];
#pragma unroll
        for (int u = 0; u < 8; u++) { const int i = i0 + u * ORD_THREADS; hv[u] = i < n ? hget(i) : 0; }
#pragma unroll
        for (int u = 0; u < 8; u++) {
          const int i = i0 + u * ORD_THREADS;
          const uint64_t key = okey(hv[u], i);
          if (i < n && (key & prefmask) == prefix) atomicAdd(&hist[(uint32_t)(key >> sh) & (nb - 1)], 1u);
        }
      }
      __syncthreads();
      const uint32_t target = (uint32_t)(K - 1) - below;
      const int per = ORD_BINS / ORD_THREADS;
      uint32_t loc = 0;
      for (int j = 0; j < per; j++) loc += hist[threadIdx.x * per + j];
      uint32_t incl = loc;
#pragma unroll
      for (int off = 1; off < 64; off <<= 1) {
        const uint32_t v = __shfl_up(incl, off);
        if ((threadIdx.x & 63) >= (unsigned)off) incl += v;
      }
      if ((threadIdx.x & 63) == 63) part[threadIdx.x >> 6] = incl;
      __syncthreads();
      for (unsigned w = 0; w < (threadIdx.x >> 6); w++) incl += part[w];
      const uint32_t excl = incl - loc;
      if (target >= excl && target < incl) {
        uint32_t run = excl;
        for (int j = 0; j < per; j++) {
          const uint32_t c = hist[threadIdx.x * per + j];
          if (target < run + c) { s_bin = threadIdx.x * per + j; s_below = run; s_cnt = c; break; }
          run += c;
        }
      }
      __syncthreads();
      const uint32_t bin = s_bin, binbelow = s_below, bincnt = s_cnt;
      __syncthreads();
      below += binbelow;
      prefix |= (uint64_t)bin << sh;
      prefmask |= (uint64_t)(nb - 1) << sh;
      bound = prefix | (sh > 0 ? ((1ULL << sh) - 1) : 0ULL);
      if (below + bincnt <= (uint32_t)cap) {
        ORD_PATH_LEVEL(lv);
        if (lv == 0) {
          uint32_t run = excl, mx = 0;
          for (int j = 0; j < per; j++) {
            const uint32_t b = threadIdx.x * per + j, c = hist[b];
            if (b <= bin) { bstart[b] = (uint16_t)run; mx = c > mx ? c : mx; }
            run += c;
          }
          if (mx > ORD_BUCKET_MAX) atomicMax(&s_fill, mx);
          __syncthreads();
          buckets = s_fill == 0;
          bk_bin = bin; bk_total = below + bincnt;
          __syncthreads();
          if (threadIdx.x == 0) s_fill = 0;
        }
        break;
      }
    }
  }
  if (buckets) {
    for (uint32_t b = threadIdx.x; b <= bk_bin; b += ORD_THREADS) hist[b] = 0;
    __syncthreads();
    for (int i0 = threadIdx.x; i0 < n; i0 += 8 * ORD_THREADS) {
      int32_t hv[8];
#pragma unroll
      for (int u = 0; u < 8; u++) { const int i = i0 + u * ORD_THREADS; hv[u] = i < n ? hget(i) : 0; }
#pragma unroll
      for (int u = 0; u < 8; u++) {
        const int i = i0 + u * ORD_THREADS;
        const uint64_t key = okey(hv[u], i);
        const uint32_t b = (uint32_t)(key >> 53);
        if (i < n && b <= bk_bin) buf[(uint32_t)bstart[b] + atomicAdd(&hist[b], 1u)] = key;
      }
    }
    __syncthreads();
    int32_t* orow = out_rows + strand * out_stride;
    for (uint32_t t = threadIdx.x; t < bk_total; t += ORD_THREADS) {
      const uint64_t key = buf[t];
      const uint32_t b = (uint32_t)(key >> 53), s0 = bstart[b], c = hist[b];
      uint32_t rank = 0;
      for (uint32_t q = 0; q < c; q += 4) {
        uint64_t o[4];
#pragma unroll
        for (int x = 0; x < 4; x++) o[x] = buf[s0 + q + (uint32_t)x < (uint32_t)cap ? s0 + q + (uint32_t)x : s0];
#pragma unroll
        for (int x = 0; x < 4; x++) rank += (q + (uint32_t)x < c && o[x] < key) ? 1u : 0u;
      }
      const uint32_t j = s0 + rank;
      if (j < (uint32_t)K) { orow[2 * j] = (int32_t)((uint32_t)(key >> 32) ^ 0x80000000u); orow[2 * j + 1] = (int32_t)(uint32_t)key; }
    }
    ORD_PATH_HOW(3);
    return;
  }
  ORD_PATH_NETWORK;
  __syncthreads();
  for (int i = threadIdx.x; i < n; i += ORD_THREADS) {
    const uint64_t key = okey(hget(i), i);
    if (key <= bound) { uint32_t slot = atomicAdd(&s_fill, 1u); if (slot < (uint32_t)cap) buf[slot] = key; }
  }
  __syncthreads();
  const uint32_t m = s_fill < (uint32_t)cap ? s_fill : (uint32_t)cap;
  uint32_t np2 = 1;
  while (np2 < m) np2 <<= 1;
  for (uint32_t j = m + threadIdx.x; j < np2; j += ORD_THREADS) buf[j] = ~0ULL;
  __syncthreads();
  for (uint32_t size = 2; size <= np2; size <<= 1) {
    for (uint32_t stride = size >> 1; stride > 0; stride >>= 1) {
      for (uint32_t t = threadIdx.x; t < (np2 >> 1); t += ORD_THREADS) {
        const uint32_t lo = 2 * t - (t & (stride - 1));
        const uint32_t hi = lo + stride;
        const bool up = ((lo & size) == 0);
        const uint64_t a = buf[lo], b = buf[hi];
        if ((a > b) == up) { buf[lo] = b; buf[hi] = a; }
      }
      __syncthreads();
    }
  }
  int32_t* orow = out_rows + strand * out_stride;
  for (int j = threadIdx.x; j < K; j += ORD_THREADS) {
    const uint64_t key = buf[j];
    orow[2 * j] = (int32_t)((uint32_t)(key >> 32) ^ 0x80000000u);
    orow[2 * j + 1] = (int32_t)(uint32_t)key;
  }
}

#ifndef MH_ORD_PAD
#define MH_ORD_PAD 0
#endif
size_t ordered_lds_bytes(int cap, int code_words, int stage_wide) {
  return (size_t)ORD_BINS * 4 + (size_t)ORD_THREADS * 4 + 16 + (size_t)cap * 8 + (size_t)(ORD_BINS + 2) * 2 + (size_t)cap * (stage_wide ? 4 : 2) +
         (code_words > 0 ? (size_t)256 * 8 + (size_t)code_words * 4 : 0) + 8 + MH_ORD_PAD;
}

__global__ void fix_status_kernel(int32_t* __restrict__ meta, int64_t nreads) {
  const int64_t i = (int64_t)blockIdx.x * blockDim.x + threadIdx.x;
  if (i >= nreads) return;
  const int32_t fs = meta[(2 * i) * META_W + 3];
  if (fs != 0 && meta[(2 * i + 1) * META_W + 3] == 0) meta[(2 * i + 1) * META_W + 3] = fs;
}

void launch_fix_status(hipStream_t st, int32_t* meta, int64_t nreads) {
  if (nreads <= 0) return;
  hipLaunchKernelGGL(fix_status_kernel, dim3((unsigned)((nreads + 255) / 256)), dim3(256), 0, st, meta, nreads);
}

void launch_ordered(hipStream_t st, const ReadDesc* descs, int64_t nstrands, int max_len_codes, int max_len, const int32_t* h32,
                    const uint8_t* store, const uint64_t* luts, int k2, int S, int cap, int32_t* out_rows, int64_t out_stride,
                    int32_t* out_meta, int64_t meta_stride, int64_t first, int64_t count) {
  if (count < 0 || first + count > nstrands) count = nstrands - first;
  if (nstrands <= 0 || count <= 0) return;
  const int code_words = max_len_codes > 0 ? (max_len_codes + 15) / 16 + 4 : 0;
  const int stage_wide = max_len - k2 + 1 > 65535 ? 1 : 0;
#ifdef MH_ORD_PATHS
  uint32_t* d_paths = nullptr;
  if (hipMalloc(&d_paths, (size_t)count * sizeof(uint32_t)) != hipSuccess) d_paths = nullptr;
  if (d_paths) (void)hipMemsetAsync(d_paths, 0, (size_t)count * sizeof(uint32_t), st);
  (void)hipStreamSynchronize(st);
  (void)hipMemcpyToSymbol(HIP_SYMBOL(g_ord_paths), &d_paths, sizeof(d_paths));
#endif
  hipLaunchKernelGGL(ordered_kernel, dim3((unsigned)count), dim3(ORD_THREADS), ordered_lds_bytes(cap, code_words, stage_wide), st, descs, nstrands, h32,
                     store, luts, code_words, stage_wide, k2, S, cap, out_rows, out_stride, out_meta, meta_stride, first);
#ifdef MH_ORD_PROF
  (void)hipStreamSynchronize(st);
  unsigned long long hp[8];
  (void)hipMemcpyFromSymbol(hp, HIP_SYMBOL(g_ord_prof), sizeof(hp));
  fprintf(stderr, "[ordered prof] cap %d lds %zu strands(one-pass) %llu  100MHz ticks/strand: stage %.1f pass1 %.1f scan %.1f fill %.1f isort %.1f out %.1f\n", cap,
          ordered_lds_bytes(cap, code_words, stage_wide), hp[7], (double)hp[0] / hp[7], (double)hp[1] / hp[7], (double)hp[2] / hp[7], (double)hp[3] / hp[7],
          (double)hp[4] / hp[7], (double)hp[5] / hp[7]);
  unsigned long long z[8] = {0, 0, 0, 0, 0, 0, 0, 0};
  (void)hipMemcpyToSymbol(HIP_SYMBOL(g_ord_prof), z, sizeof(z));
#endif
#ifdef MH_ORD_PATHS
  {
    std::vector<uint32_t> h_paths((size_t)count, 0u);
    if (d_paths) (void)hipMemcpyAsync(h_paths.data(), d_paths, (size_t)count * sizeof(uint32_t), hipMemcpyDeviceToHost, st);
    (void)hipStreamSynchronize(st);
    if (d_paths) (void)hipFree(d_paths);
    std::string line;
    line.reserve((size_t)count * 4 + 96);
    char tmp[96];
    snprintf(tmp, sizeof(tmp), "[ordered paths] first %lld count %lld cap %d S %d codes:", (long long)first, (long long)count, cap, S);
    line += tmp;
    for (uint32_t c : h_paths) { snprintf(tmp, sizeof(tmp), " %03x", c & 0xFFFu); line += tmp; }
    fprintf(stderr, "%s\n", line.c_str());
  }
#endif
}

}
```

Measured before the change: 447,300.

## Defer ordered sketch kernel to side stream and copy metadata early

Adds an opt-in mode that runs the ordered-sketch kernel on the side stream after index build, waiting on it only before overlap kernels. By default it starts an async device-to-host copy of read metadata right after the status fix kernel, overlapping it with the ordered kernel instead of doing a synchronous copy later. To support this, fix_status now writes sequence lengths into metadata. Many API entry points gain drain calls to keep state consistent, which adds bookkeeping and risks ordering bugs.

```diff
diff --git a/mhap_amd/csrc/kernels.hpp b/mhap_amd/csrc/kernels.hpp
--- a/mhap_amd/csrc/kernels.hpp
+++ b/mhap_amd/csrc/kernels.hpp
@@ -74,7 +74,7 @@
 constexpr int W1_JUMP_NA = MH_W1_JUMP_NA;
 inline int w1_jump_tables(int H) { return W1_JUMP_NA + ((H + 1) >> XS_JUMP_LOG2) / W1_JUMP_NA + 1; }
 void build_xorshift_jump_tables(int na, int nq, uint64_t* out);
-void launch_fix_status(hipStream_t st, int32_t* meta, int64_t nreads);
+void launch_fix_status(hipStream_t st, int32_t* meta, const ReadDesc* descs, int64_t nreads);
 size_t ordered_lds_bytes(int cap, int code_words, int stage_wide);
 void launch_ordered(hipStream_t st, const ReadDesc* descs, int64_t nstrands, int max_len_codes, int max_len, const int32_t* h32,
                     const uint8_t* store, const uint64_t* luts, int k2, int S, int cap, int32_t* out_rows, int64_t out_stride,
diff --git a/mhap_amd/csrc/mhap_capi.hip b/mhap_amd/csrc/mhap_capi.hip
--- a/mhap_amd/csrc/mhap_capi.hip
+++ b/mhap_amd/csrc/mhap_capi.hip
@@ -86,6 +86,10 @@
   int join_wide = 2;
   hipStream_t mh_stream = nullptr;
   hipEvent_t ev_mh_fork = nullptr, ev_mh_join = nullptr, ev_ix_fork = nullptr, ev_ix_join = nullptr;
+  hipEvent_t ev_ord_done = nullptr, ev_fix_done = nullptr;
+  bool ord_pending = false;
+  TimedLaunch ord_timed{}; bool ord_timed_set = false;
+  struct { int64_t rows = 0; const int32_t* src = nullptr; bool on = false; } meta_early;
   bool inv_ready = false; int64_t inv_ne = 0;
   uint64_t index_gen = 0;
   bool ph_ready = false; int64_t ph_ne = 0;
@@ -179,6 +183,20 @@
   HIPCHK(h, hipStreamSynchronize(h->stream));
   time_collect(h);
   return MHAP_OK;
+}
+
+void drain_ordered(mhap_handle* h) {
+  if (!h || !h->ord_pending) return;
+  (void)hipSetDevice(h->device);
+  (void)hipEventSynchronize(h->ev_ord_done);
+  h->ord_pending = false;
+  if (h->ord_timed_set) {
+    float ms = 0.f;
+    const TimedLaunch& t = h->ord_timed;
+    if (hipEventElapsedTime(&ms, t.a, t.b) == hipSuccess) { h->ktimes.ms[t.kind] += ms; h->ktimes.launches[t.kind]++; }
+    h->free_events.emplace_back(t.a, t.b);
+    h->ord_timed_set = false;
+  }
 }
 
 void build_pass_min(const std::vector<double>& tbl, int S, double threshold, std::vector<int32_t>& pm) {
@@ -320,6 +338,8 @@
 }
 
 int ensure_inverted_index(mhap_handle* h, hipStream_t st = nullptr, int64_t ne_override = -1);
+static void* pinned_io(mhap_handle* h, size_t bytes);
+static void defer_delay_sleep(void* ms) { std::this_thread::sleep_for(std::chrono::milliseconds((intptr_t)ms)); }
 int fill_ids(mhap_handle* h, int64_t first, const int64_t* ids, int64_t n) {
   h->ids.resize((size_t)(first + 2 * n)); h->fwd.resize((size_t)(first + 2 * n));
   for (int64_t i = 0; i < n; i++) {
@@ -337,7 +357,7 @@
 
 
 int sketch_staged(mhap_handle* h, int32_t* d_minhash, int64_t mh_stride, int32_t* d_ordered, int64_t ord_stride, int32_t* d_meta,
-                  int64_t eager_index_entries = 0, bool eager_exchange = false, bool eager_first = false) {
+                  int64_t eager_index_entries = 0, bool eager_exchange = false, bool eager_first = false, bool own_add = false) {
   const int64_t n = h->st_n;
   if (n <= 0) { if (eager_exchange) { const int rx = dist_eager_begin(h, 0, nullptr, false); if (rx < 0) return rx; } return MHAP_OK; }
   HPROF("sketch_staged begin");
@@ -472,8 +492,8 @@
     HIPCHK(h, hipMemcpyAsync(lens, ctr + 4, 16, hipMemcpyDeviceToHost, h->stream));
     { const int rs = sync_stream(h); if (rs != MHAP_OK) return rs; }
     HPROF("sketch: list lengths back");
-    const hipStream_t ost = h->stream;
-    auto do_ordered = [&](int64_t first, int64_t count) -> int {
+    auto do_ordered = [&](int64_t first, int64_t count, hipStream_t side = nullptr) -> int {
+      const hipStream_t ost = side ? side : h->stream;
       time_begin(h, MHAP_K_ORDERED, ost);
       launch_ordered(ost, dd, nstr, max_len_codes, B.max_len, h->h32.as<int32_t>(), h->store.as<uint8_t>(), h->hash_luts.as<uint64_t>(), k2, S, h->ord_cap,
                      ord_rows, ord_stride, meta_rows, META_W, first, count);
@@ -519,26 +539,49 @@
     }
     time_end_at(h, t_mh);
     DBGSYNC(h, "minhash");
-    launch_fix_status(h->stream, meta_rows, nb);
+    launch_fix_status(h->stream, meta_rows, dd, nb);
     if (eager_x) { const int rxm = dist_eager_minhash(h, h->stream, mh_rows, meta_rows); if (rxm != MHAP_OK) return rxm; }
+    const bool last_group = &B == &plan.back();
+    const bool meta_early = last_group && own_add && h->pend_ids.n > 0;
+    if (meta_early) HIPCHK(h, hipEventRecord(h->ev_fix_done, h->stream));
+    const bool eager_index = eager_index_entries > 0 && last_group && !getenv("MHAP_NO_EAGER_INDEX");
+    const bool defer_on = []() { const char* e = getenv("MHAP_ORDERED_DEFER"); return e && atoi(e) != 0; }();
+    const bool defer = defer_on && eager_index && own_add && !h->external && h->dist == nullptr && !eager_exchange && !ordered_done && nstr - ord_pre > 0;
     bool eager_launched = false;
-    if (eager_index_entries > 0 && &B == &plan.back() && !getenv("MHAP_NO_EAGER_INDEX")) {
+    if (eager_index) {
       HIPCHK(h, hipEventRecord(h->ev_ix_fork, h->stream));
       HIPCHK(h, hipStreamWaitEvent(h->mh_stream, h->ev_ix_fork, 0));
-      const int rce = ensure_inverted_index(h, h->mh_stream, eager_index_entries);
+      const int rce = ensure_inverted_index(h, defer ? h->stream : h->mh_stream, eager_index_entries);
       if (rce != MHAP_OK) return rce;
-      HIPCHK(h, hipEventRecord(h->ev_ix_join, h->mh_stream));
+      if (defer) {
+        const int delay_ms = []() { const char* e = getenv("MHAP_ORDERED_DEFER_DELAY_MS"); return e ? atoi(e) : 0; }();
+        if (delay_ms > 0) HIPCHK(h, hipLaunchHostFunc(h->mh_stream, defer_delay_sleep, (void*)(intptr_t)std::min(delay_ms, 1000)));
+        (void)do_ordered(ord_pre, nstr - ord_pre, h->mh_stream);
+        h->ord_timed = h->pending.back(); h->pending.pop_back(); h->ord_timed_set = true;
+        HIPCHK(h, hipEventRecord(h->ev_ord_done, h->mh_stream));
+        h->ord_pending = true;
+        ordered_done = true;
+      }
+      if (!defer) HIPCHK(h, hipEventRecord(h->ev_ix_join, h->mh_stream));
       eager_launched = true;
     }
     if (!ordered_done) (void)do_ordered(ord_pre, nstr - ord_pre);
     DBGSYNC(h, "ordered");
     HIPCHK(h, hipGetLastError());
-    if (eager_launched) HIPCHK(h, hipStreamWaitEvent(h->stream, h->ev_ix_join, 0));
+    if (eager_launched && !defer) HIPCHK(h, hipStreamWaitEvent(h->stream, h->ev_ix_join, 0));
     HPROF("sketch: all launched");
     if (&B == &plan.back() && h->pend_ids.n > 0 && !h->pend_ids.done) {
       const int rf = fill_ids(h, h->pend_ids.first, h->pend_ids.ids, h->pend_ids.n);
       if (rf != MHAP_OK) { (void)sync_stream(h); return rf; }
       h->pend_ids.done = true;
+    }
+    if (meta_early) {
+      const size_t mbytes = (size_t)(2 * n) * META_W * 4;
+      if (void* pin = pinned_io(h, mbytes)) {
+        HIPCHK(h, hipStreamWaitEvent(h->copy_stream, h->ev_fix_done, 0));
+        HIPCHK(h, hipMemcpyAsync(pin, d_meta, mbytes, hipMemcpyDeviceToHost, h->copy_stream));
+        h->meta_early.rows = 2 * n; h->meta_early.src = d_meta; h->meta_early.on = true;
+      }
     }
     int rc = sync_stream(h);
     if (rc != MHAP_OK) return rc;
@@ -584,7 +627,9 @@
 int mirror_meta(mhap_handle* h, const int32_t* d_meta, int64_t first, int64_t count) {
   int32_t* m = (int32_t*)pinned_io(h, (size_t)count * META_W * 4);
   if (!m) return fail(h, MHAP_E_HIP, "cannot allocate pinned host memory");
-  HIPCHK(h, hipMemcpy(m, d_meta + first * META_W, (size_t)count * META_W * 4, hipMemcpyDeviceToHost));
+  const bool early = h->meta_early.on && h->meta_early.src == d_meta + first * META_W && h->meta_early.rows == count;
+  if (h->meta_early.on) { h->meta_early.on = false; HIPCHK(h, hipStreamSynchronize(h->copy_stream)); }
+  if (!early) HIPCHK(h, hipMemcpy(m, d_meta + first * META_W, (size_t)count * META_W * 4, hipMemcpyDeviceToHost));
   if ((int64_t)h->seqlen.size() < first + count) { h->seqlen.resize((size_t)(first + count)); h->status.resize((size_t)(first + count)); }
   for (int64_t e = 0; e < count; e++) { h->seqlen[(size_t)(first + e)] = m[(size_t)e * META_W + 2]; h->status[(size_t)(first + e)] = (uint8_t)m[(size_t)e * META_W + 3]; }
   return MHAP_OK;
@@ -753,6 +798,7 @@
   const int64_t per_lane = 3LL * (2LL * S + 2);
   const char* omode = getenv("MHAP_OVERLAP");
   const bool lane_only = omode && strcmp(omode, "lane") == 0;
+  if (!use_index || lane_only) drain_ordered(h);
   { const char* jw = getenv("MHAP_JOIN_WIDE"); h->join_wide = !jw ? 2 : (jw[0] == '0' ? 0 : (jw[0] == '1' ? 1 : 2)); }
   { const char* jm = getenv("MHAP_JOIN_MODE"); h->join_mode = !jm ? 0 : (strcmp(jm, "alone") == 0 ? 1 : (strcmp(jm, "pair") == 0 ? 2 : (strcmp(jm, "team") == 0 ? 3 : 0))); }
   const int ntu = (ne + CAND_TM - 1) / CAND_TM;
@@ -766,7 +812,14 @@
   PostStage post; post.h = h; post.qs = &qs; post.sink = sink; post.user = user;
 #define SCHK(expr) do { const hipError_t _e = (expr); if (_e != hipSuccess) return leave(fail(h, _e == hipErrorOutOfMemory ? MHAP_E_NOMEM : MHAP_E_HIP, std::string(#expr) + ": " + hipGetErrorString(_e))); } while (0)
   auto leave = [&](int code) { const int pr = post.drain(); h->stats.matches_found += post.matches; post.matches = 0;
+                               drain_ordered(h);
                                if (code == MHAP_OK && pr != MHAP_OK) return fail(h, pr, post.err); return code; };
+  bool ord_waited = false;
+  auto ord_wait = [&]() -> hipError_t {
+    if (!h->ord_pending || ord_waited) return hipSuccess;
+    ord_waited = true;
+    return hipStreamWaitEvent(h->stream, h->ev_ord_done, 0);
+  };
   int64_t chunk_no = 0;
   const char* ppe = getenv("MHAP_SEARCH_PIPELINE");
   const bool pipeline = !(ppe && ppe[0] == '0');
@@ -912,6 +965,7 @@
       const bool prune = pe ? pe[0] == '1' : (int64_t)ncand >= 16LL * nq;
       const uint16_t *ph = nullptr, *qph = nullptr;
       if (prune) {
+        SCHK(ord_wait());
         time_begin(h, MHAP_K_OVERLAP);
         if (!(h->ph_ready && h->ph_ne == h->n_entries)) {
           SCHK(h->poshist.ensure((size_t)h->n_entries * POSHIST_BINS * 2));
@@ -931,6 +985,7 @@
         time_end(h);
         SCHK(hipGetLastError());
       }
+      SCHK(ord_wait());
       time_begin(h, MHAP_K_OVERLAP);
       launch_overlap_join(h->stream, 0, shape, jg.blocks, jg.chunk, h->cand.as<Candidate>(), ctr + levels[0].in_count, (unsigned long long)cand_cap, h->d_ordered, 2LL * S, h->d_meta,
                           qs.d_ordered, qs.ord_stride, qs.d_meta, sp, h->score_tbl.as<double>(), recbuf.as<DevRecord>(), ctr + 1,
@@ -974,6 +1029,7 @@
       while (spread < 64 && (int64_t)nslow * spread * 2 <= (int64_t)h->num_cus * 4 * 64) spread *= 2;
       const int oblocks = (int)std::max<int64_t>(1, std::min<int64_t>(ovl_max_blocks, ((int64_t)nslow * spread + OVL_THREADS - 1) / OVL_THREADS));
       SCHK(h->ovl_scratch.ensure((size_t)oblocks * OVL_THREADS / (size_t)spread * (size_t)per_lane * 4));
+      SCHK(ord_wait());
       time_begin(h, MHAP_K_OVERLAP);
       launch_overlap(h->stream, oblocks, slow_list ? slow_list : (use_join ? h->slow_cand.as<Candidate>() : h->cand.as<Candidate>()), slow_list ? slow_count_ptr : (use_join ? ctr + 5 : ctr + 0),
                      use_join ? (unsigned long long)ncand : (unsigned long long)cand_cap, h->d_ordered, 2LL * S, h->d_meta,
@@ -1007,6 +1063,7 @@
 
 namespace mhap {
 HandleView handle_view(mhap_handle* h) {
+  drain_ordered(h);
   HandleView v;
   v.device = h->device; v.stream = h->stream; v.num_cus = h->num_cus; v.Hrow = h->Hrow; v.S = h->P.ordered_sketch_size; v.k = h->P.kmer_size; v.min_olap_length = h->P.min_olap_length;
   v.max_shift = h->P.max_shift;
@@ -1016,6 +1073,7 @@
   return v;
 }
 int internal_stage_packed(mhap_handle* h, const ReadDesc* descs, const int64_t* ids, int64_t n, const void* packed, size_t bytes) {
+  drain_ordered(h);
   (void)hipSetDevice(h->device);
   h->st_descs.assign(descs, descs + n);
   h->st_ids.assign(ids, ids + n);
@@ -1032,6 +1090,7 @@
                                  const int64_t* d_ids_dev, int64_t m, int to_self, mhap_record_sink sink, void* user);
 
 int internal_sketch_queries(mhap_handle* h, const char* bases, const int64_t* offsets, const int32_t* lengths, int64_t n, void* d_mh, void* d_od, void* d_mt) {
+  drain_ordered(h);
   for (int64_t i = 0; i < n; i++) if (lengths[i] < 0) return fail(h, MHAP_E_INVALID, "negative read length");
   return sketch_into(h, bases, offsets, lengths, n, true, (int32_t*)d_mh, h->Hrow, (int32_t*)d_od, 2LL * h->P.ordered_sketch_size, (int32_t*)d_mt);
 }
@@ -1093,7 +1152,8 @@
   if (hipStreamCreateWithFlags(&h->mh_stream, hipStreamNonBlocking) != hipSuccess || hipStreamCreateWithFlags(&h->copy_stream, hipStreamNonBlocking) != hipSuccess ||
       hipEventCreateWithFlags(&h->ev_mh_fork, hipEventDisableTiming) != hipSuccess ||
       hipEventCreateWithFlags(&h->ev_mh_join, hipEventDisableTiming) != hipSuccess || hipEventCreateWithFlags(&h->ev_ix_fork, hipEventDisableTiming) != hipSuccess ||
-      hipEventCreateWithFlags(&h->ev_ix_join, hipEventDisableTiming) != hipSuccess) { seterr("cannot create the side streams"); mhap_destroy(h); return MHAP_E_HIP; }
+      hipEventCreateWithFlags(&h->ev_ix_join, hipEventDisableTiming) != hipSuccess || hipEventCreateWithFlags(&h->ev_ord_done, hipEventDisableTiming) != hipSuccess ||
+      hipEventCreateWithFlags(&h->ev_fix_done, hipEventDisableTiming) != hipSuccess) { seterr("cannot create the side streams"); mhap_destroy(h); return MHAP_E_HIP; }
   h->Hrow = std::max(1, P.num_hashes);
   int cap = 1; while (cap < P.ordered_sketch_size) cap <<= 1;
   h->ord_cap = cap;
@@ -1117,6 +1177,7 @@
 
 void mhap_destroy(mhap_handle* h) {
   if (!h) return;
+  drain_ordered(h);
   (void)hipSetDevice(h->device);
   if (h->stream) (void)hipStreamSynchronize(h->stream);
   if (h->dist) { mhap_dist_release(h->dist); h->dist = nullptr; }
@@ -1137,6 +1198,8 @@
   if (h->ev_mh_join) (void)hipEventDestroy(h->ev_mh_join);
   if (h->ev_ix_fork) (void)hipEventDestroy(h->ev_ix_fork);
   if (h->ev_ix_join) (void)hipEventDestroy(h->ev_ix_join);
+  if (h->ev_ord_done) (void)hipEventDestroy(h->ev_ord_done);
+  if (h->ev_fix_done) (void)hipEventDestroy(h->ev_fix_done);
   if (h->mh_stream) (void)hipStreamDestroy(h->mh_stream);
   if (h->own_stream) (void)hipStreamDestroy(h->own_stream);
   delete h;
@@ -1147,6 +1210,7 @@
 int mhap_set_filter(mhap_handle* h, const int64_t* hashes, const double* fractions, int64_t n, double filter_cutoff, double offset,
                     double range, int no_tf) {
   if (!h) return MHAP_E_INVALID;
+  drain_ordered(h);
   (void)hipSetDevice(h->device);
   if (n <= 0 && !hashes) { h->ft = FilterTable{nullptr, nullptr, 0, 0, 0, 0, range}; return MHAP_OK; }
   if (offset < 0.0 || offset >= 1.0) return fail(h, MHAP_E_INVALID, "Offset can only be between 0 and 1.0.");
@@ -1182,6 +1246,7 @@
 
 int mhap_set_filter_whitelist(mhap_handle* h, const int64_t* hashes, int64_t n, int64_t size_bloom, int32_t mode) {
   if (!h) return MHAP_E_INVALID;
+  drain_ordered(h);
   if (mode < 0 || mode > 2) return fail(h, MHAP_E_INVALID, "Unknown removeUnique option.");
   if (mode == 0) { h->ft.bloom = nullptr; h->ft.bloom_bits = 0; h->ft.bloom_k = 0; h->ft.bloom_mode = 0; return MHAP_OK; }
   if (!h->ft.enabled) return fail(h, MHAP_E_STATE, "set the k-mer filter (mhap_set_filter) before its whitelist");
@@ -1211,6 +1276,7 @@
 
 int mhap_index_add_reads(mhap_handle* h, const char* bases, const int64_t* offsets, const int32_t* lengths, const int64_t* ids, int64_t n) {
   if (!h) return MHAP_E_INVALID;
+  drain_ordered(h);
   (void)hipSetDevice(h->device);
   if (n > 0 && (!bases || !offsets || !lengths || !ids)) return leave_collective_add(h, fail(h, MHAP_E_INVALID, "null argument"));
   if (n <= 0) return leave_collective_add(h, MHAP_OK);
@@ -1243,6 +1309,7 @@
 
 int mhap_stage_reads(mhap_handle* h, const char* bases, const int64_t* offsets, const int32_t* lengths, const int64_t* ids, int64_t n) {
   if (!h || n < 0 || (n > 0 && (!bases || !offsets || !lengths || !ids))) return h ? fail(h, MHAP_E_INVALID, "null argument") : MHAP_E_INVALID;
+  drain_ordered(h);
   (void)hipSetDevice(h->device);
   for (int64_t i = 0; i < n; i++) if (lengths[i] < 0) return fail(h, MHAP_E_INVALID, "negative read length");
   h->st_ids.assign(ids, ids + n);
@@ -1260,6 +1327,7 @@
 
 int mhap_index_add_staged(mhap_handle* h) {
   if (!h) return MHAP_E_INVALID;
+  drain_ordered(h);
   (void)hipSetDevice(h->device);
   const int64_t n = h->st_n;
   if (n <= 0 || (int64_t)h->st_ids.size() != n) return leave_collective_add(h, fail(h, MHAP_E_STATE, "no staged reads (call mhap_stage_reads first)"));
@@ -1275,14 +1343,17 @@
   const bool eager_exchange = h->dist != nullptr && dist_eager_wanted(h);
   h->pend_ids.first = first; h->pend_ids.n = n; h->pend_ids.ids = h->st_ids.data(); h->pend_ids.done = false;
   rc = sketch_staged(h, h->d_minhash + first * h->Hrow, h->Hrow, h->d_ordered + first * 2LL * S, 2LL * S, h->d_meta + first * META_W,
-                     likely_last ? after : 0, eager_exchange, first == 0);
+                     likely_last ? after : 0, eager_exchange, first == 0, true);
   if (rc != MHAP_OK) {
+    drain_ordered(h);
+    if (h->meta_early.on) { h->meta_early.on = false; (void)hipStreamSynchronize(h->copy_stream); }
     h->pend_ids.n = 0; h->pend_ids.done = false;
     h->ids.resize((size_t)first); h->fwd.resize((size_t)first);
     return rc;
   }
   const bool built = h->inv_ready && h->inv_ne == after;
   rc = finish_add(h, first, h->st_ids.data(), n);
+  if (rc != MHAP_OK) drain_ordered(h);
   if (rc == MHAP_OK && built) h->inv_ready = true;
   if (rc == MHAP_OK && eager_exchange) dist_eager_commit(h);
   return rc;
@@ -1290,6 +1361,7 @@
 
 int mhap_sketch_staged_device(mhap_handle* h, void* d_minhash, void* d_ordered, void* d_meta) {
   if (!h || !d_minhash || !d_ordered || !d_meta) return h ? fail(h, MHAP_E_INVALID, "null argument") : MHAP_E_INVALID;
+  drain_ordered(h);
   (void)hipSetDevice(h->device);
   if (h->st_n <= 0) return fail(h, MHAP_E_STATE, "no staged reads (call mhap_stage_reads first)");
   return sketch_staged(h, (int32_t*)d_minhash, h->Hrow, (int32_t*)d_ordered, 2LL * h->P.ordered_sketch_size, (int32_t*)d_meta);
@@ -1298,6 +1370,7 @@
 int mhap_sketch_batch(mhap_handle* h, const char* bases, const int64_t* offsets, const int32_t* lengths, int64_t n, int32_t* minhash,
                       int32_t* ordered, int32_t* ordered_size, uint8_t* status) {
   if (!h) return MHAP_E_INVALID;
+  drain_ordered(h);
   if (n <= 0) return MHAP_OK;
   if (!bases || !offsets || !lengths) return fail(h, MHAP_E_INVALID, "null argument");
   (void)hipSetDevice(h->device);
@@ -1338,6 +1411,7 @@
 int mhap_index_add_sketches(mhap_handle* h, const int64_t* ids, const uint8_t* is_fwd, const int32_t* seq_length, const int32_t* minhash,
                             const int32_t* ordered, const int32_t* ordered_size, const int32_t* ordered_seqlen, int64_t m) {
   if (!h) return MHAP_E_INVALID;
+  drain_ordered(h);
   if (m <= 0) return MHAP_OK;
   if (!ids || !is_fwd || !seq_length || !minhash || !ordered || !ordered_size || !ordered_seqlen) return fail(h, MHAP_E_INVALID, "null argument");
   (void)hipSetDevice(h->device);
@@ -1381,6 +1455,7 @@
 int mhap_index_export(mhap_handle* h, int64_t first, int64_t count, int64_t* ids, uint8_t* is_fwd, int32_t* seq_length, int32_t* minhash,
                       int32_t* ordered, int32_t* ordered_size, int32_t* ordered_seqlen, uint8_t* status) {
   if (!h) return MHAP_E_INVALID;
+  drain_ordered(h);
   if (first < 0 || count < 0 || first + count > h->n_entries) return fail(h, MHAP_E_INVALID, "export range outside the index");
   if (count == 0) return MHAP_OK;
   (void)hipSetDevice(h->device);
@@ -1402,6 +1477,7 @@
 
 int mhap_index_clear(mhap_handle* h) {
   if (!h) return MHAP_E_INVALID;
+  drain_ordered(h);
   h->n_entries = 0; h->external = false; h->inv_ready = false; h->ph_ready = false; h->reserve_reads = 0; h->index_gen++;
   h->ids.clear(); h->fwd.clear(); h->seqlen.clear(); h->status.clear();
   h->d_minhash = h->own_minhash.as<int32_t>(); h->d_ordered = h->own_ordered.as<int32_t>(); h->d_meta = h->own_meta.as<int32_t>();
@@ -1411,6 +1487,7 @@
 
 int mhap_index_prepare(mhap_handle* h) {
   if (!h) return MHAP_E_INVALID;
+  drain_ordered(h);
   (void)hipSetDevice(h->device);
   if (h->n_entries == 0) return MHAP_OK;
   const int rc = ensure_inverted_index(h);
@@ -1421,6 +1498,7 @@
 int mhap_sketch_reads_device(mhap_handle* h, const char* bases, const int64_t* offsets, const int32_t* lengths, int64_t n, void* d_minhash,
                              void* d_ordered, void* d_meta) {
   if (!h) return MHAP_E_INVALID;
+  drain_ordered(h);
   if (n <= 0) return MHAP_OK;
   if (!bases || !offsets || !lengths || !d_minhash || !d_ordered || !d_meta) return fail(h, MHAP_E_INVALID, "null argument");
   (void)hipSetDevice(h->device);
@@ -1430,6 +1508,7 @@
 
 int mhap_index_set_device(mhap_handle* h, const int64_t* ids, const uint8_t* is_fwd, void* d_minhash, void* d_ordered, void* d_meta, int64_t m) {
   if (!h) return MHAP_E_INVALID;
+  drain_ordered(h);
   if (m < 0 || (m > 0 && (!ids || !is_fwd || !d_minhash || !d_ordered || !d_meta))) return fail(h, MHAP_E_INVALID, "null argument");
   if (m > (int64_t)INT32_MAX / 2) return fail(h, MHAP_E_INVALID, "index too large for 32-bit entry indices");
   (void)hipSetDevice(h->device);
@@ -1483,6 +1562,7 @@
 int mhap_find_matches_reads(mhap_handle* h, const char* bases, const int64_t* offsets, const int32_t* lengths, const int64_t* ids, int64_t n,
                             mhap_record_sink sink, void* user) {
   if (!h) return MHAP_E_INVALID;
+  drain_ordered(h);
   if (n <= 0) return MHAP_OK;
   if (!bases || !offsets || !lengths || !ids) return fail(h, MHAP_E_INVALID, "null argument");
   (void)hipSetDevice(h->device);
@@ -1592,16 +1672,17 @@
 }
 
 int mhap_get_stats(mhap_handle* h, mhap_stats* out) { if (!h || !out) return MHAP_E_INVALID; *out = h->stats; return MHAP_OK; }
-int mhap_get_kernel_times(mhap_handle* h, mhap_kernel_times* out) { if (!h || !out) return MHAP_E_INVALID; *out = h->ktimes; return MHAP_OK; }
-int mhap_reset_kernel_times(mhap_handle* h) { if (!h) return MHAP_E_INVALID; h->ktimes = mhap_kernel_times{}; return MHAP_OK; }
+int mhap_get_kernel_times(mhap_handle* h, mhap_kernel_times* out) { if (!h || !out) return MHAP_E_INVALID; drain_ordered(h); *out = h->ktimes; return MHAP_OK; }
+int mhap_reset_kernel_times(mhap_handle* h) { if (!h) return MHAP_E_INVALID; drain_ordered(h); h->ktimes = mhap_kernel_times{}; return MHAP_OK; }
 int mhap_set_stream(mhap_handle* h, void* hip_stream) {
   if (!h) return MHAP_E_INVALID;
+  drain_ordered(h);
   (void)hipSetDevice(h->device);
   (void)hipStreamSynchronize(h->stream);
   h->stream = hip_stream ? (hipStream_t)hip_stream : h->own_stream;
   return MHAP_OK;
 }
-int mhap_synchronize(mhap_handle* h) { if (!h) return MHAP_E_INVALID; (void)hipSetDevice(h->device); return sync_stream(h); }
+int mhap_synchronize(mhap_handle* h) { if (!h) return MHAP_E_INVALID; drain_ordered(h); (void)hipSetDevice(h->device); return sync_stream(h); }
 
 }
 
diff --git a/mhap_amd/csrc/sketch_kernels.hip b/mhap_amd/csrc/sketch_kernels.hip
--- a/mhap_amd/csrc/sketch_kernels.hip
+++ b/mhap_amd/csrc/sketch_kernels.hip
@@ -2233,16 +2233,19 @@
          (code_words > 0 ? (size_t)256 * 8 + (size_t)code_words * 4 : 0) + 8 + MH_ORD_PAD;
 }
 
-__global__ void fix_status_kernel(int32_t* __restrict__ meta, int64_t nreads) {
+__global__ void fix_status_kernel(int32_t* __restrict__ meta, const ReadDesc* __restrict__ descs, int64_t nreads) {
   const int64_t i = (int64_t)blockIdx.x * blockDim.x + threadIdx.x;
   if (i >= nreads) return;
+  const int32_t len = descs[i].length;
+  meta[(2 * i) * META_W + 2] = len;
+  meta[(2 * i + 1) * META_W + 2] = len;
   const int32_t fs = meta[(2 * i) * META_W + 3];
   if (fs != 0 && meta[(2 * i + 1) * META_W + 3] == 0) meta[(2 * i + 1) * META_W + 3] = fs;
 }
 
-void launch_fix_status(hipStream_t st, int32_t* meta, int64_t nreads) {
+void launch_fix_status(hipStream_t st, int32_t* meta, const ReadDesc* descs, int64_t nreads) {
   if (nreads <= 0) return;
-  hipLaunchKernelGGL(fix_status_kernel, dim3((unsigned)((nreads + 255) / 256)), dim3(256), 0, st, meta, nreads);
+  hipLaunchKernelGGL(fix_status_kernel, dim3((unsigned)((nreads + 255) / 256)), dim3(256), 0, st, meta, descs, nreads);
 }
 
 void launch_ordered(hipStream_t st, const ReadDesc* descs, int64_t nstrands, int max_len_codes, int max_len, const int32_t* h32,
```

New measurement: 446,100, median of 2. No clear change (-0.3%).
